# andimarafioti/faster-qwen3-tts

Hardware: AMD Instinct MI355X
Metric: real-time factor (audio s / wall s), Qwen3-TTS-12Hz-0.6B voice-clone streaming chunk_size=8; p50 TTFA in ttfa_ms_p50 (higher is better)
Workload: dtype bf16

## Files before the change

faster-qwen3-tts_amd/csrc/decode_kernels.cuh:

```cuda
#pragma once
#include "fq3_common.cuh"
#include <initializer_list>

namespace fq3 {

enum { PRO_PLAIN = 0, PRO_NORM = 1, PRO_COMBINE = 2 };
enum { EPI_STORE = 0, EPI_RESIDUAL = 1, EPI_SWIGLU = 2 };

constexpr int kHeadDim = 128;
constexpr int kKeysPerTile = 64;
constexpr int kMaxWorkers = 8;
constexpr int kPartStride = kHeadDim + 4;


struct GemvArgs {
    const void* W; int N; int K;
    const void* x;
    const void* norm_w; float eps;
    const void* bias;
    void* y;
    const void* res;
    void* xn_out;
    int up_off;
    const float* part; int n_part; int rep;
    const void* x2; void* y2; const void* res2; size_t part_stride2;
};

struct CombineRegs {
    f32x4 oa[kMaxWorkers], ob[kMaxWorkers];
    float pm[kMaxWorkers], pl[kMaxWorkers];
};
__device__ __forceinline__ void combine_load(CombineRegs& c, const float* part, int e0, int rep, int n_part) {
    const int head = e0 / kHeadDim, d0 = e0 - head * kHeadDim;
    const int g = head / rep, hh = head - g * rep;
    const float* p0 = part + ((size_t)(g * kMaxWorkers) * rep + hh) * kPartStride;
    const size_t sstride = (size_t)rep * kPartStride;
#pragma unroll
    for (int s = 0; s < kMaxWorkers; ++s) {
        const float* ps = p0 + (s < n_part ? s : 0) * sstride;
        c.oa[s] = *reinterpret_cast<const f32x4*>(ps + d0);
        c.ob[s] = *reinterpret_cast<const f32x4*>(ps + d0 + 4);
        c.pm[s] = ps[kHeadDim]; c.pl[s] = ps[kHeadDim + 1];
    }
}
template <typename T>
__device__ __forceinline__ void combine_finish(CombineRegs& c, int n_part, float (&f)[8]) {
#pragma unroll
    for (int s = 1; s < kMaxWorkers; ++s)
        if (s >= n_part) { c.pm[s] = -1e30f; c.pl[s] = 0.f; }
    float Mx = c.pm[0];
#pragma unroll
    for (int s = 1; s < kMaxWorkers; ++s) Mx = fmaxf(Mx, c.pm[s]);
    f32x4 na = f32x4{0.f, 0.f, 0.f, 0.f}, nb = na;
    float den = 0.f;
#pragma unroll
    for (int s = 0; s < kMaxWorkers; ++s) {
        const float w = __expf(c.pm[s] - Mx);
        na += c.oa[s] * w; nb += c.ob[s] * w; den = fmaf(w, c.pl[s], den);
    }
    const float inv = 1.0f / den;
    f[0] = na.x * inv; f[1] = na.y * inv; f[2] = na.z * inv; f[3] = na.w * inv;
    f[4] = nb.x * inv; f[5] = nb.y * inv; f[6] = nb.z * inv; f[7] = nb.w * inv;
#pragma unroll
    for (int i = 0; i < 8; i += 2) DT<T>::rnd2(f[i], f[i + 1]);
}

template <int NCH, int EPI> struct MaxRows {
    static constexpr int NR = EPI == EPI_SWIGLU ? 2 : 1;
    static constexpr int v = NCH >= 12 ? 1 : (NCH >= 6 ? (2 / NR) : 2);
};

inline int gemv_chunks(int K, int most) {
    const int need = (K + 511) / 512;
    for (int n : {1, 2, 4, 6, 12}) if (need <= n && n <= most) return n;
    return 0;
}

template <typename T, int NCH, int PRO, int EPI, bool NT, int M = 1, int R = 1>
__device__ __forceinline__ void gemv_body(const GemvArgs& a) {
    constexpr int NR = (EPI == EPI_SWIGLU) ? 2 : 1;
    extern __shared__ __attribute__((aligned(16))) float xs[];
    const int tid = threadIdx.x, wave = tid >> 6, lane = tid & 63;
    const int K = a.K;
    const T* W = reinterpret_cast<const T*>(a.W);
    const int row0 = (blockIdx.x * 4 + wave) * R;

    Raw8<T> xraw[M][NCH], nraw[NCH];
    CombineRegs cr[M];
    if constexpr (PRO == PRO_COMBINE) {
        const int e0 = tid * 8 < K ? tid * 8 : 0;
#pragma unroll
        for (int m = 0; m < M; ++m) combine_load(cr[m], a.part + (size_t)m * a.part_stride2, e0, a.rep, a.n_part);
    } else {
#pragma unroll
        for (int j = 0; j < NCH; ++j) {
            const int off = j * 512 + lane * 8, offc = off < K ? off : 0;
#pragma unroll
            for (int m = 0; m < M; ++m) ldraw<false>(xraw[m][j], reinterpret_cast<const T*>(m == 0 ? a.x : a.x2) + offc);
            if constexpr (PRO == PRO_NORM) ldraw<false>(nraw[j], reinterpret_cast<const T*>(a.norm_w) + offc);
        }
    }
    __builtin_amdgcn_sched_barrier(0);

    Raw8<T> raw[NR][R][NCH];
#pragma unroll
    for (int h = 0; h < NR; ++h)
#pragma unroll
        for (int r = 0; r < R; ++r) {
            const int row = row0 + r < a.N ? row0 + r : a.N - 1;
            const T* wr = W + (size_t)(row + h * a.up_off) * K;
#pragma unroll
            for (int j = 0; j < NCH; ++j) {
                const int off = j * 512 + lane * 8;
                ldraw<NT>(raw[h][r][j], wr + (off < K ? off : 0));
            }
        }
    float resv[M][R], biasv[R];
#pragma unroll
    for (int r = 0; r < R; ++r) {
        const int row = row0 + r < a.N ? row0 + r : a.N - 1;
#pragma unroll
        for (int m = 0; m < M; ++m) {
            const T* rp = reinterpret_cast<const T*>(m == 0 ? a.res : a.res2);
            resv[m][r] = 0.f;
            if constexpr (EPI == EPI_RESIDUAL) resv[m][r] = DT<T>::ld(rp + row);
        }
        const T* bp = a.bias ? reinterpret_cast<const T*>(a.bias) + row : W;
        const float bv = DT<T>::ld(bp);
        biasv[r] = a.bias ? bv : 0.f;
    }
    __builtin_amdgcn_sched_barrier(0);

    float xr[M][NCH][8];
    if constexpr (PRO == PRO_COMBINE) {
#pragma unroll
        for (int m = 0; m < M; ++m) {
            float f[8];
            combine_finish<T>(cr[m], a.n_part, f);
            if (tid * 8 < K) {
                float* d = xs + (size_t)m * K + tid * 8;
                reinterpret_cast<f32x4*>(d)[0] = f32x4{f[0], f[1], f[2], f[3]};
                reinterpret_cast<f32x4*>(d)[1] = f32x4{f[4], f[5], f[6], f[7]};
            }
        }
        __syncthreads();
#pragma unroll
        for (int m = 0; m < M; ++m)
#pragma unroll
            for (int j = 0; j < NCH; ++j) {
                const int off = j * 512 + lane * 8, offc = off < K ? off : 0;
                const float z = off < K ? 1.f : 0.f;
                const f32x4 lo = *reinterpret_cast<const f32x4*>(xs + (size_t)m * K + offc) * z;
                const f32x4 hi = *reinterpret_cast<const f32x4*>(xs + (size_t)m * K + offc + 4) * z;
                xr[m][j][0] = lo.x; xr[m][j][1] = lo.y; xr[m][j][2] = lo.z; xr[m][j][3] = lo.w;
                xr[m][j][4] = hi.x; xr[m][j][5] = hi.y; xr[m][j][6] = hi.z; xr[m][j][7] = hi.w;
            }
    } else {
#pragma unroll
        for (int m = 0; m < M; ++m) {
#pragma unroll
            for (int j = 0; j < NCH; ++j) {
                if (j * 512 + lane * 8 >= K) zero(xraw[m][j]);
                unpack(xraw[m][j], xr[m][j]);
            }
            if constexpr (PRO == PRO_NORM) {
                float ss = 0.f;
#pragma unroll
                for (int j = 0; j < NCH; ++j)
#pragma unroll
                    for (int i = 0; i < 8; ++i) ss = fmaf(xr[m][j][i], xr[m][j][i], ss);
                ss = wave_sum(ss);
                const float rs = 1.0f / sqrtf(ss / (float)K + a.eps);
#pragma unroll
                for (int j = 0; j < NCH; ++j) {
                    float nw[8];
                    unpack(nraw[j], nw);
#pragma unroll
                    for (int i = 0; i < 8; i += 2) {
                        float u = xr[m][j][i] * rs, v = xr[m][j][i + 1] * rs;
                        DT<T>::rnd2(u, v);
                        u *= nw[i]; v *= nw[i + 1];
                        DT<T>::rnd2(u, v);
                        xr[m][j][i] = u; xr[m][j][i + 1] = v;
                    }
                }
            }
        }
    }

    float acc[M][R][NR];
#pragma unroll
    for (int m = 0; m < M; ++m)
#pragma unroll
        for (int r = 0; r < R; ++r)
#pragma unroll
            for (int h = 0; h < NR; ++h) {
                float s = 0.f;
#pragma unroll
                for (int j = 0; j < NCH; ++j) s = dot8<T>(raw[h][r][j], xr[m][j], s);
                acc[m][r][h] = s;
            }
#pragma unroll
    for (int m = 0; m < M; ++m)
#pragma unroll
        for (int r = 0; r < R; ++r)
#pragma unroll
            for (int h = 0; h < NR; ++h) acc[m][r][h] = wave_sum(acc[m][r][h]);
#pragma unroll
    for (int r = 0; r < R; ++r) {
        const int row = row0 + r;
#pragma unroll
        for (int m = 0; m < M; ++m) {
            float v;
            if constexpr (EPI == EPI_SWIGLU) {
                const float g = DT<T>::rnd(acc[m][r][0]);
                const float u = DT<T>::rnd(acc[m][r][NR - 1]);
                const float sg = DT<T>::rnd(g / (1.0f + expf(-g)));
                v = sg * u;
            } else {
                v = DT<T>::rnd(acc[m][r][0] + biasv[r]);
                if constexpr (EPI == EPI_RESIDUAL) v = v + resv[m][r];
            }
            if (lane == 0 && row < a.N) DT<T>::st(reinterpret_cast<T*>(m == 0 ? a.y : a.y2) + row, v);
        }
    }
    if (a.xn_out && blockIdx.x == 0 && wave == 0) {
        T* o = reinterpret_cast<T*>(a.xn_out);
#pragma unroll
        for (int j = 0; j < NCH; ++j) {
            const int off = j * 512 + lane * 8;
            if (off < K) DT<T>::st8(o + off, xr[0][j]);
        }
    }
}

template <typename T, int NCH, int PRO, int EPI, bool NT, int M = 1, int R = 1>
__global__ __launch_bounds__(256) void gemv_kernel(GemvArgs a) { gemv_body<T, NCH, PRO, EPI, NT, M, R>(a); }

struct AttnArgs {
    const void* qkv;
    const void* q_norm_w; const void* k_norm_w; float eps;
    const float* cos_row; const float* sin_row;
    void* kcache; void* vcache; int max_seq;
    const int* table; int blk_stride;
    const int* pos_ptr; int pos_imm; int n_pad;
    const int* done_ptr;
    int n_kv; float* part; float scale;
    int rep; void* out;
};

template <typename T, int REP, bool PAGED>
__device__ __forceinline__ void attn_decode_body(const AttnArgs& a) {
    constexpr int HD = kHeadDim, KS = kKeysPerTile, NG = KS / 16;
    const int g = blockIdx.x, s = blockIdx.y, S = gridDim.y;
    __shared__ float qs[REP][HD];
    __shared__ float knew[HD], vnew[HD];
    __shared__ float wo[4][REP][HD];
    __shared__ float wm[4][REP], wl[4][REP];
    const int tid = threadIdx.x, wave = tid >> 6, lane = tid & 63;
    const int sub = lane >> 4, c = lane & 15;
    const T* qkv = reinterpret_cast<const T*>(a.qkv);
    const int q_dim = a.n_kv * REP * HD, kv_dim = a.n_kv * HD;
    T* kc = reinterpret_cast<T*>(a.kcache) + (PAGED ? (size_t)g * KS * HD : (size_t)g * a.max_seq * HD);
    T* vc = reinterpret_cast<T*>(a.vcache) + (PAGED ? (size_t)g * KS * HD : (size_t)g * a.max_seq * HD);
    const int n_tiles = (a.max_seq + KS - 1) / KS;
    auto block_of = [&](int tile) -> int {
        if constexpr (PAGED) return a.table[tile < n_tiles ? tile : n_tiles - 1];
        else return 0;
    };
    int blk = block_of(s), blk_next = block_of(s + S);

    Raw8<T> kr[NG], vr[NG];
    auto issue_tile = [&](int tile, int b) {
#pragma unroll
        for (int i = 0; i < NG; ++i) {
            const int kt = (i * 4 + wave) * 4 + sub;
            size_t off;
            if constexpr (PAGED) off = (size_t)b * a.blk_stride + (size_t)kt * HD;
            else { int key = tile * KS + kt; key = key < a.max_seq ? key : a.max_seq - 1; off = (size_t)key * HD; }
            ldraw<false>(kr[i], kc + off + c * 8);
            ldraw<false>(vr[i], vc + off + c * 8);
        }
    };
    if constexpr (!PAGED) issue_tile(s, 0);
    constexpr int NV = (REP + 2 + 3) / 4;
    float px0[NV], px1[NV], pw0[NV], pw1[NV];
#pragma unroll
    for (int i = 0; i < NV; ++i) {
        const int vec = wave + 4 * i < REP + 2 ? wave + 4 * i : REP + 1;
        const T* src = vec < REP ? qkv + (size_t)(g * REP + vec) * HD
                     : (vec == REP ? qkv + q_dim + (size_t)g * HD : qkv + q_dim + kv_dim + (size_t)g * HD);
        px0[i] = DT<T>::ld(src + lane); px1[i] = DT<T>::ld(src + lane + 64);
        const T* w = reinterpret_cast<const T*>(vec < REP ? a.q_norm_w : a.k_norm_w);
        pw0[i] = DT<T>::ld(w + lane); pw1[i] = DT<T>::ld(w + lane + 64);
    }
    const float cs = a.cos_row[lane], sn = a.sin_row[lane];
    const int pos = a.pos_ptr ? *a.pos_ptr : a.pos_imm;
    const int done_word = *(a.done_ptr ? a.done_ptr : reinterpret_cast<const int*>(a.cos_row));
    const bool loop_done = a.done_ptr != nullptr && done_word != 0;
    if constexpr (PAGED) issue_tile(s, blk);
    __builtin_amdgcn_sched_barrier(0);

    const int t_pos = pos / KS;
    const bool owner = (t_pos % S) == s;
    const bool may_append = owner && !loop_done;
    size_t new_off = (size_t)pos * HD;
    if constexpr (PAGED) new_off = (size_t)block_of(t_pos) * a.blk_stride + (size_t)(pos - t_pos * KS) * HD;
#pragma unroll
    for (int i = 0; i < NV; ++i) {
        const int vec = wave + 4 * i;
        if (vec >= REP + 2) continue;
        float x0 = px0[i], x1 = px1[i];
        if (vec <= REP) {
            const float ss = wave_sum(fmaf(x0, x0, x1 * x1));
            const float rs = 1.0f / sqrtf(ss / (float)HD + a.eps);
            const float n0 = DT<T>::rnd(pw0[i] * DT<T>::rnd(x0 * rs));
            const float n1 = DT<T>::rnd(pw1[i] * DT<T>::rnd(x1 * rs));
            x0 = DT<T>::rnd(DT<T>::rnd(n0 * cs) + DT<T>::rnd(-n1 * sn));
            x1 = DT<T>::rnd(DT<T>::rnd(n1 * cs) + DT<T>::rnd(n0 * sn));
        }
        if (vec < REP) { qs[vec][lane] = x0; qs[vec][lane + 64] = x1; }
        else {
            float* dst = vec == REP ? knew : vnew;
            dst[lane] = x0; dst[lane + 64] = x1;
            if (may_append) {
                T* cp = (vec == REP ? kc : vc) + new_off;
                DT<T>::st(cp + lane, x0); DT<T>::st(cp + lane + 64, x1);
            }
        }
    }
    __syncthreads();

    float qr[REP][8];
#pragma unroll
    for (int h = 0; h < REP; ++h)
#pragma unroll
        for (int i = 0; i < 8; ++i) qr[h][i] = qs[h][c * 8 + i];

    float m[REP], l[REP], o[REP][8];
#pragma unroll
    for (int h = 0; h < REP; ++h) {
        m[h] = -1e30f; l[h] = 0.f;
#pragma unroll
        for (int i = 0; i < 8; ++i) o[h][i] = 0.f;
    }
    auto step = [&](const float (&kf)[8], const float (&vf)[8], bool valid) {
#pragma unroll
        for (int h = 0; h < REP; ++h) {
            float sc = 0.f;
#pragma unroll
            for (int i = 0; i < 8; ++i) sc = fmaf(qr[h][i], kf[i], sc);
            sc = row16_sum(sc);
            sc = valid ? sc * a.scale : -INFINITY;
            const float mn = fmaxf(m[h], sc);
            const float al = __expf(m[h] - mn);
            const float p = __expf(sc - mn);
            l[h] = fmaf(l[h], al, p);
#pragma unroll
            for (int i = 0; i < 8; ++i) o[h][i] = fmaf(o[h][i], al, valid ? p * vf[i] : 0.f);
            m[h] = mn;
        }
    };
    for (int tile = s; tile * KS < pos || tile == s; tile += S) {
        if (tile != s) { blk = blk_next; issue_tile(tile, blk); }
        blk_next = block_of(tile + S);
#pragma unroll
        for (int i = 0; i < NG; ++i) {
            const int key = tile * KS + (i * 4 + wave) * 4 + sub;
            float kf[8], vf[8];
            unpack(kr[i], kf); unpack(vr[i], vf);
            step(kf, vf, key >= a.n_pad && key < pos);
        }
    }
    {
        float kf[8], vf[8];
#pragma unroll
        for (int i = 0; i < 8; ++i) { kf[i] = knew[c * 8 + i]; vf[i] = vnew[c * 8 + i]; }
        step(kf, vf, owner && wave == 0 && sub == 0 && pos >= a.n_pad);
    }
#pragma unroll
    for (int h = 0; h < REP; ++h) {
        const float M = xrow_max(m[h]);
        const float w = __expf(m[h] - M);
        l[h] = xrow_sum(l[h] * w);
#pragma unroll
        for (int i = 0; i < 8; ++i) o[h][i] = xrow_sum(o[h][i] * w);
        m[h] = M;
    }
    if (sub == 0) {
#pragma unroll
        for (int h = 0; h < REP; ++h) {
#pragma unroll
            for (int i = 0; i < 8; ++i) wo[wave][h][c * 8 + i] = o[h][i];
            if (c == 0) { wm[wave][h] = m[h]; wl[wave][h] = l[h]; }
        }
    }
    __syncthreads();
    for (int e = tid; e < REP * HD; e += 256) {
        const int h = e / HD, d = e - h * HD;
        float M = fmaxf(fmaxf(wm[0][h], wm[1][h]), fmaxf(wm[2][h], wm[3][h]));
        float num = 0.f, den = 0.f;
#pragma unroll
        for (int w = 0; w < 4; ++w) {
            const float ww = __expf(wm[w][h] - M);
            num = fmaf(ww, wo[w][h][d], num);
            den = fmaf(ww, wl[w][h], den);
        }
        float* p = a.part + (((size_t)g * kMaxWorkers + s) * REP + h) * kPartStride;
        p[d] = num;
        if (d == 0) { p[HD] = M; p[HD + 1] = den; }
    }
}

template <typename T, int REP, bool PAGED>
__global__ __launch_bounds__(256) void attn_decode_kernel(AttnArgs a) { attn_decode_body<T, REP, PAGED>(a); }

template <typename T>
__device__ __forceinline__ void attn_pred_body(const AttnArgs& a, int head) {
    constexpr int HD = kHeadDim;
    const int g = head / a.rep, hh = head - g * a.rep;
    const int lane = threadIdx.x & 63, sub = lane >> 4, c = lane & 15;
    const int pos = a.pos_imm;
    const T* qkv = reinterpret_cast<const T*>(a.qkv);
    const int q_dim = a.n_kv * a.rep * HD, kv_dim = a.n_kv * HD;
    T* kc = reinterpret_cast<T*>(a.kcache) + (size_t)g * a.max_seq * HD;
    T* vc = reinterpret_cast<T*>(a.vcache) + (size_t)g * a.max_seq * HD;
    Raw8<T> qraw, knraw, vnraw, qwraw, kwraw, kr[4], vr[4];
    ldraw<false>(qraw, qkv + (size_t)head * HD + c * 8);
    ldraw<false>(knraw, qkv + q_dim + (size_t)g * HD + c * 8);
    ldraw<false>(vnraw, qkv + q_dim + kv_dim + (size_t)g * HD + c * 8);
    ldraw<false>(qwraw, reinterpret_cast<const T*>(a.q_norm_w) + c * 8);
    ldraw<false>(kwraw, reinterpret_cast<const T*>(a.k_norm_w) + c * 8);
    const f32x4 cs0 = *reinterpret_cast<const f32x4*>(a.cos_row + ((c * 8) & 63)), cs1 = *reinterpret_cast<const f32x4*>(a.cos_row + ((c * 8 + 4) & 63));
    const f32x4 sn0 = *reinterpret_cast<const f32x4*>(a.sin_row + ((c * 8) & 63)), sn1 = *reinterpret_cast<const f32x4*>(a.sin_row + ((c * 8 + 4) & 63));
#pragma unroll
    for (int i = 0; i < 4; ++i) {
        int key = i * 4 + sub;
        key = key < a.max_seq ? key : a.max_seq - 1;
        ldraw<false>(kr[i], kc + (size_t)key * HD + c * 8);
        ldraw<false>(vr[i], vc + (size_t)key * HD + c * 8);
    }
    __builtin_amdgcn_sched_barrier(0);
    const float sgn = c < 8 ? -1.f : 1.f;
    const float cs[8] = {cs0.x, cs0.y, cs0.z, cs0.w, cs1.x, cs1.y, cs1.z, cs1.w};
    const float sn[8] = {sgn * sn0.x, sgn * sn0.y, sgn * sn0.z, sgn * sn0.w, sgn * sn1.x, sgn * sn1.y, sgn * sn1.z, sgn * sn1.w};
    auto norm_rope = [&](const Raw8<T>& raw, const Raw8<T>& wraw, float (&out)[8]) {
        float x[8], w[8];
        unpack(raw, x); unpack(wraw, w);
        float ss = 0.f;
#pragma unroll
        for (int i = 0; i < 8; ++i) ss = fmaf(x[i], x[i], ss);
        ss = row16_sum(ss);
        const float rs = 1.0f / sqrtf(ss / (float)HD + a.eps);
#pragma unroll
        for (int i = 0; i < 8; i += 2) {
            float u = x[i] * rs, v = x[i + 1] * rs;
            DT<T>::rnd2(u, v);
            u *= w[i]; v *= w[i + 1];
            DT<T>::rnd2(u, v);
            x[i] = u; x[i + 1] = v;
        }
#pragma unroll
        for (int i = 0; i < 8; i += 2) {
            float a0 = x[i] * cs[i], a1 = x[i + 1] * cs[i + 1];
            float b0 = row16_xor8(x[i]) * sn[i], b1 = row16_xor8(x[i + 1]) * sn[i + 1];
            DT<T>::rnd2(a0, a1); DT<T>::rnd2(b0, b1);
            float r0 = a0 + b0, r1 = a1 + b1;
            DT<T>::rnd2(r0, r1);
            out[i] = r0; out[i + 1] = r1;
        }
    };
    float qr[8], knew[8], vnew[8];
    norm_rope(qraw, qwraw, qr);
    norm_rope(knraw, kwraw, knew);
    unpack(vnraw, vnew);
    if (hh == 0 && sub == 0) {
        DT<T>::st8(kc + (size_t)pos * HD + c * 8, knew);
        DT<T>::st8(vc + (size_t)pos * HD + c * 8, vnew);
    }
    float sc[5];
#pragma unroll
    for (int i = 0; i < 4; ++i) {
        float kf[8], s = 0.f;
        unpack(kr[i], kf);
#pragma unroll
        for (int d = 0; d < 8; ++d) s = fmaf(qr[d], kf[d], s);
        s = row16_sum(s);
        sc[i] = (i * 4 + sub < pos) ? s * a.scale : -INFINITY;
    }
    {
        float s = 0.f;
#pragma unroll
        for (int d = 0; d < 8; ++d) s = fmaf(qr[d], knew[d], s);
        s = row16_sum(s);
        sc[4] = sub == 0 ? s * a.scale : -INFINITY;
    }
    const float mx = wave_max(fmaxf(fmaxf(fmaxf(sc[0], sc[1]), fmaxf(sc[2], sc[3])), sc[4]));
    float p[5], lsum = 0.f, o[8];
#pragma unroll
    for (int i = 0; i < 5; ++i) { p[i] = __expf(sc[i] - mx); lsum += p[i]; }
    lsum = wave_sum(lsum) * (1.0f / 16.0f);
#pragma unroll
    for (int d = 0; d < 8; ++d) o[d] = p[4] * vnew[d];
#pragma unroll
    for (int i = 0; i < 4; ++i) {
        float vf[8];
        if (!(i * 4 + sub < pos)) zero(vr[i]);
        unpack(vr[i], vf);
#pragma unroll
        for (int d = 0; d < 8; ++d) o[d] = fmaf(p[i], vf[d], o[d]);
    }
    const float inv = 1.0f / lsum;
#pragma unroll
    for (int d = 0; d < 8; ++d) o[d] = xrow_sum(o[d]) * inv;
    if (sub == 0) DT<T>::st8(reinterpret_cast<T*>(a.out) + (size_t)head * HD + c * 8, o);
}

template <typename T>
__device__ __forceinline__ void attn_pred_body(const AttnArgs& a) { attn_pred_body<T>(a, (int)blockIdx.x); }

template <typename T, int REP>
__device__ __forceinline__ void attn_pred_group_body(const AttnArgs& a, int g) {
    constexpr int HD = kHeadDim;
    const int lane = threadIdx.x & 63, sub = lane >> 4, c = lane & 15;
    const int pos = a.pos_imm;
    const T* qkv = reinterpret_cast<const T*>(a.qkv);
    const int q_dim = a.n_kv * REP * HD, kv_dim = a.n_kv * HD;
    T* kc = reinterpret_cast<T*>(a.kcache) + (size_t)g * a.max_seq * HD;
    T* vc = reinterpret_cast<T*>(a.vcache) + (size_t)g * a.max_seq * HD;
    Raw8<T> qraw[REP], knraw, vnraw, qwraw, kwraw, kr[4], vr[4];
#pragma unroll
    for (int h = 0; h < REP; ++h) ldraw<false>(qraw[h], qkv + (size_t)(g * REP + h) * HD + c * 8);
    ldraw<false>(knraw, qkv + q_dim + (size_t)g * HD + c * 8);
    ldraw<false>(vnraw, qkv + q_dim + kv_dim + (size_t)g * HD + c * 8);
    ldraw<false>(qwraw, reinterpret_cast<const T*>(a.q_norm_w) + c * 8);
    ldraw<false>(kwraw, reinterpret_cast<const T*>(a.k_norm_w) + c * 8);
    const f32x4 cs0 = *reinterpret_cast<const f32x4*>(a.cos_row + ((c * 8) & 63)), cs1 = *reinterpret_cast<const f32x4*>(a.cos_row + ((c * 8 + 4) & 63));
    const f32x4 sn0 = *reinterpret_cast<const f32x4*>(a.sin_row + ((c * 8) & 63)), sn1 = *reinterpret_cast<const f32x4*>(a.sin_row + ((c * 8 + 4) & 63));
#pragma unroll
    for (int i = 0; i < 4; ++i) {
        int key = i * 4 + sub;
        key = key < pos ? key : 0;
        ldraw<false>(kr[i], kc + (size_t)key * HD + c * 8);
        ldraw<false>(vr[i], vc + (size_t)key * HD + c * 8);
    }
    __builtin_amdgcn_sched_barrier(0);
    const float sgn = c < 8 ? -1.f : 1.f;
    const float cs[8] = {cs0.x, cs0.y, cs0.z, cs0.w, cs1.x, cs1.y, cs1.z, cs1.w};
    const float sn[8] = {sgn * sn0.x, sgn * sn0.y, sgn * sn0.z, sgn * sn0.w, sgn * sn1.x, sgn * sn1.y, sgn * sn1.z, sgn * sn1.w};
    auto norm_rope = [&](const Raw8<T>& raw, const Raw8<T>& wraw, float (&out)[8]) {
        float x[8], w[8];
        unpack(raw, x); unpack(wraw, w);
        float ss = 0.f;
#pragma unroll
        for (int i = 0; i < 8; ++i) ss = fmaf(x[i], x[i], ss);
        ss = row16_sum(ss);
        const float rs = 1.0f / sqrtf(ss / (float)HD + a.eps);
#pragma unroll
        for (int i = 0; i < 8; i += 2) {
            float u = x[i] * rs, v = x[i + 1] * rs;
            DT<T>::rnd2(u, v);
            u *= w[i]; v *= w[i + 1];
            DT<T>::rnd2(u, v);
            x[i] = u; x[i + 1] = v;
        }
#pragma unroll
        for (int i = 0; i < 8; i += 2) {
            float a0 = x[i] * cs[i], a1 = x[i + 1] * cs[i + 1];
            float b0 = row16_xor8(x[i]) * sn[i], b1 = row16_xor8(x[i + 1]) * sn[i + 1];
            DT<T>::rnd2(a0, a1); DT<T>::rnd2(b0, b1);
            float r0 = a0 + b0, r1 = a1 + b1;
            DT<T>::rnd2(r0, r1);
            out[i] = r0; out[i + 1] = r1;
        }
    };
    float knew[8], vnew[8];
    norm_rope(knraw, kwraw, knew);
    unpack(vnraw, vnew);
    if (sub == 0) {
        DT<T>::st8(kc + (size_t)pos * HD + c * 8, knew);
        DT<T>::st8(vc + (size_t)pos * HD + c * 8, vnew);
    }
    float kf[4][8], vf[4][8];
#pragma unroll
    for (int i = 0; i < 4; ++i) {
        unpack(kr[i], kf[i]);
        if (!(i * 4 + sub < pos)) zero(vr[i]);
        unpack(vr[i], vf[i]);
    }
#pragma unroll
    for (int h = 0; h < REP; ++h) {
        float qr[8];
        norm_rope(qraw[h], qwraw, qr);
        float sc[5];
#pragma unroll
        for (int i = 0; i < 4; ++i) {
            float s = 0.f;
#pragma unroll
            for (int d = 0; d < 8; ++d) s = fmaf(qr[d], kf[i][d], s);
            s = row16_sum(s);
            sc[i] = (i * 4 + sub < pos) ? s * a.scale : -INFINITY;
        }
        {
            float s = 0.f;
#pragma unroll
            for (int d = 0; d < 8; ++d) s = fmaf(qr[d], knew[d], s);
            s = row16_sum(s);
            sc[4] = sub == 0 ? s * a.scale : -INFINITY;
        }
        const float mx = wave_max(fmaxf(fmaxf(fmaxf(sc[0], sc[1]), fmaxf(sc[2], sc[3])), sc[4]));
        float p[5], lsum = 0.f, o[8];
#pragma unroll
        for (int i = 0; i < 5; ++i) { p[i] = __expf(sc[i] - mx); lsum += p[i]; }
        lsum = wave_sum(lsum) * (1.0f / 16.0f);
#pragma unroll
        for (int d = 0; d < 8; ++d) o[d] = p[4] * vnew[d];
#pragma unroll
        for (int i = 0; i < 4; ++i)
#pragma unroll
            for (int d = 0; d < 8; ++d) o[d] = fmaf(p[i], vf[i][d], o[d]);
        const float inv = 1.0f / lsum;
#pragma unroll
        for (int d = 0; d < 8; ++d) o[d] = xrow_sum(o[d]) * inv;
        if (sub == 0) DT<T>::st8(reinterpret_cast<T*>(a.out) + (size_t)(g * REP + h) * HD + c * 8, o);
    }
}

template <typename T>
__global__ __launch_bounds__(64) void attn_pred_kernel(AttnArgs a) { attn_pred_body<T>(a); }

template <typename T>
__global__ __launch_bounds__(256) void rmsnorm_kernel(const T* x, const T* w, T* y, int K, float eps) {
    __shared__ float red[8];
    float ss = 0.f;
    for (int e = threadIdx.x; e < K; e += 256) { const float v = DT<T>::ld(x + e); ss = fmaf(v, v, ss); }
    ss = block_sum<4>(ss, red);
    const float rs = 1.0f / sqrtf(ss / (float)K + eps);
    for (int e = threadIdx.x; e < K; e += 256)
        DT<T>::st(y + e, DT<T>::ld(w + e) * DT<T>::rnd(DT<T>::ld(x + e) * rs));
}

template <typename T>
__global__ void copy_kernel(T* dst, const T* src, int n) {
    const int i = blockIdx.x * blockDim.x + threadIdx.x;
    if (i < n) dst[i] = src[i];
}

struct DecodeState {
    int token, frame, pos, gen_step, done;
    int text_open;
    int min_new, max_new, trailing_len, noise_frames, eos_id, max_seq, sup_lo, sup_hi;
    float t_temperature; int t_top_k; float t_top_p; int t_do_sample; float t_rep_penalty;
    float p_temperature; int p_top_k; float p_top_p; int p_do_sample;
    const void* trailing_text; const void* tts_pad; const void* talker_noise; const void* pred_noise;
    const void* past_hidden_init;
    int n_pad, rope_delta;
};

struct TeacherForcing { const int* forced; int* decisions; };

__device__ __forceinline__ int forced_or(const TeacherForcing* tf, int slot, int tok) {
    if (!tf) return tok;
    const int* forced = gptr(tf->forced); int* dec = gptr(tf->decisions);
    if (dec && threadIdx.x == 0) dec[slot] = tok;
    return forced ? forced[slot] : tok;
}

template <typename T>
__device__ __forceinline__ void frame_begin_body(DecodeState* st, const T* codec_emb, const T* past_hidden, T* ph_hold,
                                                 T* pred_in, int* codes, unsigned char* seen, int H, int G) {
    const int done = st->done;
    if (done == 1) return;
    const int tok = st->token;
    if (tok == st->eos_id || st->frame >= st->max_new) {
        __syncthreads();
        if (threadIdx.x == 0) st->done = 1;
        return;
    }
    if (st->text_open && st->gen_step >= st->trailing_len) {
        if (done == 0) {
            for (int e = threadIdx.x; e < H; e += 256) ph_hold[e] = past_hidden[e];
            __syncthreads();
            if (threadIdx.x == 0) st->done = 2;
        }
        return;
    }
    if (done == 2) {
        past_hidden = ph_hold;
        __syncthreads();
        if (threadIdx.x == 0) st->done = 0;
    }
    if (threadIdx.x == 0) { codes[(size_t)st->frame * G] = tok; seen[tok] = 1; }
    for (int e = threadIdx.x; e < H; e += 256) {
        pred_in[e] = past_hidden[e];
        pred_in[H + e] = codec_emb[(size_t)tok * H + e];
    }
}
template <typename T>
__global__ __launch_bounds__(256) void frame_begin_kernel(DecodeState* st, const T* codec_emb, const T* past_hidden, T* ph_hold,
                                                          T* pred_in, int* codes, unsigned char* seen, int H, int G) {
    frame_begin_body<T>(st, codec_emb, past_hidden, ph_hold, pred_in, codes, seen, H, G);
}

struct EmbTables { const void* t[32]; };

template <typename T, int G>
__device__ __forceinline__ void embed_sum_body(DecodeState* st, const EmbTables& tabs, const int* codes, T* x, int H,
                                               const float* cos_tab, const float* sin_tab, int rope_len,
                                               int rope_delta, float* rope_now) {
    const int done = st->done, frame = st->frame, pos = st->pos, gen_step = st->gen_step;
    const int trailing_len = st->trailing_len, max_seq = st->max_seq;
    const T* trailing = gptr(reinterpret_cast<const T*>(st->trailing_text));
    const T* pad = gptr(reinterpret_cast<const T*>(st->tts_pad));
    if (done) return;
    if (pos >= max_seq - 1) {
        __syncthreads();
        if (threadIdx.x == 0) { st->frame = frame + 1; st->done = 1; }
        return;
    }
    int ids[G];
#pragma unroll
    for (int gI = 0; gI < G; ++gI) ids[gI] = codes[(size_t)frame * G + gI];
    if (threadIdx.x < kHeadDim) {
        int rp = pos + rope_delta;
        rp = rp < 0 ? 0 : (rp >= rope_len ? rope_len - 1 : rp);
        const int i = threadIdx.x & 63;
        rope_now[threadIdx.x] = threadIdx.x < 64 ? cos_tab[(size_t)rp * 64 + i] : sin_tab[(size_t)rp * 64 + i];
    }
    const T* text = gen_step < trailing_len ? trailing + (size_t)gen_step * H : pad;
    for (int e0 = threadIdx.x * 8; e0 < H; e0 += 256 * 8) {
        Raw8<T> r[G], tr;
#pragma unroll
        for (int gI = 0; gI < G; ++gI) ldraw<false>(r[gI], reinterpret_cast<const T*>(tabs.t[gI]) + (size_t)ids[gI] * H + e0);
        ldraw<false>(tr, text + e0);
        float sum[8], f[8];
        unpack(r[0], sum);
#pragma unroll
        for (int gI = 1; gI < G; ++gI) {
            unpack(r[gI], f);
#pragma unroll
            for (int i = 0; i < 8; ++i) sum[i] += f[i];
        }
        unpack(tr, f);
#pragma unroll
        for (int i = 0; i < 8; ++i) DT<T>::st(x + e0 + i, DT<T>::rnd(sum[i]) + f[i]);
    }
}
template <typename T, int G>
__global__ __launch_bounds__(256) void embed_sum_kernel(DecodeState* st, EmbTables tabs, const int* codes, T* x, int H,
                                                        const float* cos_tab, const float* sin_tab, int rope_len,
                                                        int rope_delta, float* rope_now) {
    embed_sum_body<T, G>(st, tabs, codes, x, H, cos_tab, sin_tab, rope_len, rope_delta, rope_now);
}

}
```

faster-qwen3-tts_amd/csrc/fq3_api.hip:

```cpp
#define FQ3_SKINNY_EXTERN
#include "fq3_ctx.h"
#include "sampler.cuh"
#include "sampler_wave.cuh"
#include "skinny_gemm.cuh"

#include <cstdio>
#include <cstdlib>
#include <cstring>
#include <map>
#include <string>
#include <type_traits>
#include <vector>

using namespace fq3;

static thread_local std::string g_err;
static int fail(int code, const std::string& m) { g_err = m; return code; }
int fq3_fail_(int code, const std::string& m) { return fail(code, m); }
#define HIPCHK(x) do { hipError_t e_ = (x); if (e_ != hipSuccess) return fail(FQ3_EHIP, std::string(#x) + ": " + hipGetErrorString(e_)); } while (0)

extern "C" const char* fq3_last_error(void) { return g_err.c_str(); }
extern "C" void fq3_set_error_(const char* msg) { g_err = msg ? msg : ""; }
extern "C" int fq3_abi_version(void) { return FQ3_ABI_VERSION; }

static int dmalloc(fq3_ctx* c, void** p, size_t bytes, bool zero = true) {
    HIPCHK(hipMalloc(p, bytes));
    if (zero) HIPCHK(hipMemset(*p, 0, bytes));
    c->allocs.push_back(*p);
    return 0;
}
int fq3_dmalloc_(fq3_ctx* c, void** p, size_t bytes) { return dmalloc(c, p, bytes, false); }

static bool dims_ok(const fq3_stack_dims& d) {
    return d.head_dim == kHeadDim && d.hidden % 8 == 0 && d.inter % 8 == 0 && d.n_heads % d.n_kv_heads == 0 &&
           (d.n_heads / d.n_kv_heads == 1 || d.n_heads / d.n_kv_heads == 2 || d.n_heads / d.n_kv_heads == 4) &&
           d.vocab <= kMaxVocab && d.vocab % 8 == 0 && d.hidden <= 2048 && d.inter <= 6144 && d.n_heads * kHeadDim <= 6144 && d.n_layers >= 1;
}

static int cfg_check(const fq3_config* cfg) {
    if (cfg->dtype != FQ3_BF16 && cfg->dtype != FQ3_F32) return fail(FQ3_EINVAL, "dtype must be FQ3_BF16 or FQ3_F32");
    if (!dims_ok(cfg->talker) || !dims_ok(cfg->predictor))
        return fail(FQ3_EUNSUPPORTED, "unsupported dims (need head_dim 128, GQA ratio 1/2/4, vocab <= 4096 and a multiple of 8, "
                                      "hidden <= 2048 and intermediate <= 6144, both multiples of 8)");
    if (cfg->num_code_groups < 2 || cfg->num_code_groups > 64) return fail(FQ3_EINVAL, "num_code_groups");
    if (cfg->max_seq_len < 8) return fail(FQ3_EINVAL, "max_seq_len");
    return 0;
}

static void pool_free_(fq3_kv_pool* p) {
    for (void* q : p->k) if (q) (void)hipFree(q);
    for (void* q : p->v) if (q) (void)hipFree(q);
    delete p;
}

static int pool_create_(const fq3_config* cfg, int n_blocks, fq3_kv_pool** out) {
    if (n_blocks < 1) return fail(FQ3_EINVAL, "fq3_kv_pool_create: n_blocks must be positive");
    fq3_kv_pool* p = new fq3_kv_pool();
    p->dtype = cfg->dtype; p->esz = cfg->dtype == FQ3_BF16 ? 2 : 4;
    p->n_layers = cfg->talker.n_layers; p->n_kv = cfg->talker.n_kv_heads; p->n_blocks = n_blocks;
    p->blk_elems = (size_t)p->n_kv * kKeysPerTile * kHeadDim;
    p->k.assign(p->n_layers, nullptr); p->v.assign(p->n_layers, nullptr);
    const size_t bytes = (size_t)n_blocks * p->blk_elems * p->esz;
    for (int i = 0; i < p->n_layers; ++i) {
        if (hipMalloc(&p->k[i], bytes) != hipSuccess || hipMalloc(&p->v[i], bytes) != hipSuccess ||
            hipMemset(p->k[i], 0, bytes) != hipSuccess || hipMemset(p->v[i], 0, bytes) != hipSuccess) {
            pool_free_(p);
            return fail(FQ3_EHIP, "fq3_kv_pool_create: allocation of " + std::to_string(2 * bytes >> 20) + " MiB per layer failed");
        }
    }
    p->free_list.resize(n_blocks);
    for (int i = 0; i < n_blocks; ++i) p->free_list[i] = n_blocks - 1 - i;
    *out = p;
    return FQ3_OK;
}

extern "C" int fq3_kv_pool_create(const fq3_config* cfg, int n_blocks, fq3_kv_pool** out) {
    if (!cfg || !out) return fail(FQ3_EINVAL, "null argument");
    if (int r = cfg_check(cfg)) return r;
    return pool_create_(cfg, n_blocks, out);
}

extern "C" int fq3_kv_pool_destroy(fq3_kv_pool* p) {
    if (!p) return FQ3_OK;
    if (p->users > 0) return fail(FQ3_ESTATE, "fq3_kv_pool_destroy: contexts are still attached");
    (void)hipDeviceSynchronize();
    pool_free_(p);
    return FQ3_OK;
}

extern "C" int fq3_kv_pool_stats(const fq3_kv_pool* p, int* n_blocks, int* n_free, int* high_water, int64_t* bytes_per_block) {
    if (!p) return fail(FQ3_EINVAL, "null pool");
    fq3_kv_pool* q = const_cast<fq3_kv_pool*>(p);
    std::lock_guard<std::mutex> lk(q->mu);
    if (n_blocks) *n_blocks = p->n_blocks;
    if (n_free) *n_free = (int)p->free_list.size();
    if (high_water) *high_water = p->in_use_high;
    if (bytes_per_block) *bytes_per_block = (int64_t)2 * p->n_layers * p->blk_elems * p->esz;
    return FQ3_OK;
}

struct KvTableVals { int v[128]; };
__global__ void kv_table_write_kernel(int* table, KvTableVals vals, int first, int count) {
    const int i = threadIdx.x;
    if (i < count) table[first + i] = vals.v[i];
}
static void table_write(fq3_ctx* c, const int* ids, int first, int count, hipStream_t s) {
    for (int o = 0; o < count; o += 128) {
        KvTableVals t{};
        const int n = std::min(128, count - o);
        for (int i = 0; i < n; ++i) t.v[i] = ids[o + i];
        hipLaunchKernelGGL(kv_table_write_kernel, dim3(1), dim3(128), 0, s, c->tk.d_table, t, first + o, n);
    }
}

static int kv_ensure(fq3_ctx* c, int n_pos, hipStream_t s, bool sync_copy);
int fq3_kv_ensure_(fq3_ctx* c, int n_pos, hipStream_t s) { return kv_ensure(c, n_pos, s, false); }
static int kv_ensure(fq3_ctx* c, int n_pos, hipStream_t s, bool sync_copy) {
    StackBufs& b = c->tk;
    int need = (std::min(n_pos, b.max_seq) + kKeysPerTile - 1) / kKeysPerTile;
    need = std::min(need, b.max_blocks);
    const int have = (int)b.blocks.size();
    if (need <= have) return 0;
    fq3_kv_pool* p = b.pool;
    {
        std::lock_guard<std::mutex> lk(p->mu);
        if ((int)p->free_list.size() < need - have) {
            char m[200];
            snprintf(m, sizeof m, "KV pool exhausted: %d more block(s) of 64 keys needed, %d free of %d", need - have, (int)p->free_list.size(), p->n_blocks);
            return fail(FQ3_ENOMEM, m);
        }
        for (int i = have; i < need; ++i) { b.blocks.push_back(p->free_list.back()); p->free_list.pop_back(); }
        p->in_use_high = std::max(p->in_use_high, p->n_blocks - (int)p->free_list.size());
    }
    if (sync_copy) HIPCHK(hipMemcpy(b.d_table + have, b.blocks.data() + have, (size_t)(need - have) * sizeof(int), hipMemcpyHostToDevice));
    else table_write(c, b.blocks.data() + have, have, need - have, s);
    return 0;
}

extern "C" int fq3_kv_release(fq3_ctx* c, int keep_positions) {
    if (!c) return fail(FQ3_EINVAL, "null ctx");
    StackBufs& b = c->tk;
    const int keep = std::max(0, std::min((int)b.blocks.size(), (keep_positions + kKeysPerTile - 1) / kKeysPerTile));
    if (keep >= (int)b.blocks.size()) return FQ3_OK;
    std::lock_guard<std::mutex> lk(b.pool->mu);
    while ((int)b.blocks.size() > keep) { b.pool->free_list.push_back(b.blocks.back()); b.blocks.pop_back(); }
    return FQ3_OK;
}

extern "C" int fq3_kv_blocks(const fq3_ctx* c) { return c ? (int)c->tk.blocks.size() : 0; }

extern "C" int fq3_kv_reserve(fq3_ctx* c, int n_positions, void* stream) {
    if (!c) return fail(FQ3_EINVAL, "null ctx");
    if (n_positions < 0) return fail(FQ3_EINVAL, "fq3_kv_reserve: negative position count");
    return fq3_kv_ensure_(c, n_positions, (hipStream_t)stream);
}

static int ctx_build(fq3_ctx* c, const fq3_config* cfg, fq3_kv_pool* pool);
static int ctx_create_(const fq3_config* cfg, fq3_kv_pool* pool, fq3_ctx** out) {
    if (!cfg || !out) return fail(FQ3_EINVAL, "null argument");
    if (int r = cfg_check(cfg)) return r;
    if (pool && (pool->dtype != cfg->dtype || pool->n_layers != cfg->talker.n_layers || pool->n_kv != cfg->talker.n_kv_heads))
        return fail(FQ3_EINVAL, "fq3_ctx_create_pooled: the pool was built for another dtype / layer count / kv head count");
    fq3_ctx* c = new fq3_ctx();
    if (int r = ctx_build(c, cfg, pool)) { const std::string m = g_err; fq3_ctx_destroy(c); g_err = m; return r; }
    *out = c;
    return FQ3_OK;
}
extern "C" int fq3_ctx_create(const fq3_config* cfg, fq3_ctx** out) { return ctx_create_(cfg, nullptr, out); }
extern "C" int fq3_ctx_create_pooled(const fq3_config* cfg, fq3_kv_pool* pool, fq3_ctx** out) {
    if (!pool) return fail(FQ3_EINVAL, "null pool");
    return ctx_create_(cfg, pool, out);
}

static int ctx_build(fq3_ctx* c, const fq3_config* cfg, fq3_kv_pool* pool) {
    c->cfg = *cfg;
    c->esz = cfg->dtype == FQ3_BF16 ? 2 : 4;
    const fq3_stack_dims &t = cfg->talker, &p = cfg->predictor;
    const int pred_seq = cfg->num_code_groups + 1;
    auto alloc_stack = [&](StackBufs& b, const fq3_stack_dims& d, int max_seq) -> int {
        b.max_seq = max_seq;
        b.workers = std::min(kMaxWorkers, (max_seq + kKeysPerTile - 1) / kKeysPerTile);
        b.k.resize(d.n_layers); b.v.resize(d.n_layers);
        const size_t bytes = (size_t)d.n_kv_heads * max_seq * kHeadDim * c->esz;
        for (int i = 0; i < d.n_layers; ++i) {
            if (int r = dmalloc(c, &b.k[i], bytes)) return r;
            if (int r = dmalloc(c, &b.v[i], bytes)) return r;
        }
        return 0;
    };
    int r;
    {
        StackBufs& b = c->tk;
        b.max_seq = cfg->max_seq_len;
        b.max_blocks = (cfg->max_seq_len + kKeysPerTile - 1) / kKeysPerTile;
        b.workers = std::min(kMaxWorkers, b.max_blocks);
        if (!pool) {
            if ((r = pool_create_(cfg, b.max_blocks, &pool))) return r;
            pool->is_private = true;
        }
        b.pool = pool;
        { std::lock_guard<std::mutex> lk(pool->mu); ++pool->users; }
        b.k = pool->k; b.v = pool->v;
        if ((r = dmalloc(c, (void**)&b.d_table, (size_t)b.max_blocks * sizeof(int)))) return r;
        if (pool->is_private && (r = kv_ensure(c, cfg->max_seq_len, nullptr, true))) return r;
    }
    if ((r = alloc_stack(c->pk, p, pred_seq))) return r;
    const int Hm = std::max(t.hidden, p.hidden), Im = std::max(t.inter, p.inter);
    const int qkvm = std::max(t.n_heads + 2 * t.n_kv_heads, p.n_heads + 2 * p.n_kv_heads) * kHeadDim;
    const int Vm = std::max(t.vocab, p.vocab);
    const int G = cfg->num_code_groups;
    const int frames = cfg->max_frames > 0 ? cfg->max_frames : 4096;
    c->cfg.max_frames = frames;
    if ((r = dmalloc(c, &c->h, (size_t)Hm * c->esz))) return r;
    if ((r = dmalloc(c, &c->h2, (size_t)Hm * c->esz))) return r;
    if ((r = dmalloc(c, &c->qkv2, (size_t)qkvm * c->esz))) return r;
    if ((r = dmalloc(c, &c->attn_out, (size_t)qkvm * c->esz))) return r;
    if ((r = dmalloc(c, &c->attn_out2, (size_t)qkvm * c->esz))) return r;
    if ((r = dmalloc(c, &c->act2, (size_t)Im * c->esz))) return r;
    if ((r = dmalloc(c, &c->pred_x2, (size_t)p.hidden * c->esz))) return r;
    if ((r = dmalloc(c, &c->xin, (size_t)Hm * c->esz))) return r;
    if ((r = dmalloc(c, &c->tmp_hidden, (size_t)Hm * c->esz))) return r;
    if ((r = dmalloc(c, &c->qkv, (size_t)qkvm * c->esz))) return r;
    if ((r = dmalloc(c, &c->act, (size_t)Im * c->esz))) return r;
    if ((r = dmalloc(c, &c->logits, (size_t)Vm * c->esz))) return r;
    if ((r = dmalloc(c, &c->past_hidden, (size_t)t.hidden * c->esz))) return r;
    if ((r = dmalloc(c, &c->ph_hold, (size_t)t.hidden * c->esz))) return r;
    if ((r = dmalloc(c, &c->pred_in, (size_t)2 * t.hidden * c->esz))) return r;
    if ((r = dmalloc(c, &c->pred_next, (size_t)t.hidden * c->esz))) return r;
    if ((r = dmalloc(c, &c->pred_x, (size_t)p.hidden * c->esz))) return r;
    if ((r = dmalloc(c, &c->plogits, (size_t)(G - 1) * p.vocab * c->esz))) return r;
    const int maxkv = std::max(t.n_kv_heads, p.n_kv_heads);
    c->part_stride = (size_t)maxkv * kMaxWorkers * 4 * kPartStride;
    if ((r = dmalloc(c, (void**)&c->part, 2 * c->part_stride * sizeof(float)))) return r;
    if ((r = dmalloc(c, (void**)&c->rope_now, 2 * 64 * sizeof(float)))) return r;
    if ((r = dmalloc(c, (void**)&c->seen_api, kMaxVocab))) return r;
    if ((r = dmalloc(c, (void**)&c->st, sizeof(DecodeState)))) return r;
    if ((r = dmalloc(c, (void**)&c->seen, kMaxVocab))) return r;
    if ((r = dmalloc(c, (void**)&c->codes, (size_t)(frames + 1) * G * sizeof(int)))) return r;
    if ((r = dmalloc(c, (void**)&c->ids64, (size_t)64 * sizeof(int64_t)))) return r;
    if ((r = dmalloc(c, (void**)&c->d_pemb, (size_t)64 * sizeof(void*)))) return r;
    HIPCHK(hipStreamCreateWithFlags(&c->cap_stream, hipStreamNonBlocking));
    return FQ3_OK;
}

extern "C" int fq3_set_option(fq3_ctx* c, const char* key, int value) {
    if (!c || !key) return fail(FQ3_EINVAL, "null argument");
    const std::string k(key);
    if (k == "weight_nt") c->opt_nt = value;
    else if (k == "pred_m2") c->opt_m2 = value;
    else if (k == "pred_attn") c->opt_pred_attn = value;
    else if (k == "rows_per_wave_max") c->opt_rmax = value;
    else if (k == "prefill_mode") c->prefill_mode = value;
    else if (k == "flash_prefill") c->opt_flash_prefill = value;
    else if (k == "flash_small") c->opt_flash_small = value;
    else if (k == "swiglu_tile") c->opt_swiglu_tile = value;
    else if (k == "packed_weights") c->opt_packed = value;
    else if (k == "skinny_gemm") c->opt_no_skinny = !value;
    else return fail(FQ3_EINVAL, "unknown option: " + k);
    fq3_graph_reset(c);
    return FQ3_OK;
}

extern "C" int fq3_graph_reset(fq3_ctx* c) {
    if (!c) return fail(FQ3_EINVAL, "null ctx");
    if (c->exec) { (void)hipGraphExecDestroy(c->exec); c->exec = nullptr; }
    if (c->graph) { (void)hipGraphDestroy(c->graph); c->graph = nullptr; }
    return FQ3_OK;
}

namespace {
struct PackedEntry { void* p; int refs; int N, K; };
std::mutex g_packed_mu;
std::map<std::pair<const void*, int>, PackedEntry> g_packed;
}
const void* fq3_packed_find_(const void* W, int kind) {
    std::lock_guard<std::mutex> lk(g_packed_mu);
    auto it = g_packed.find({W, kind});
    return it == g_packed.end() ? nullptr : it->second.p;
}
int fq3_packed_acquire_(const void* W, int N, int K, int kind) {
    if (!W || !skinny_pack_ok(N, K) || (kind == 1 && (N / 2) % 8) || (kind == 2 && N % 512)) return FQ3_EUNSUPPORTED;
    std::lock_guard<std::mutex> lk(g_packed_mu);
    auto it = g_packed.find({W, kind});
    if (it != g_packed.end()) {
        if (it->second.N != N || it->second.K != K) return fail(FQ3_EINVAL, "a matrix is bound with two different shapes");
        ++it->second.refs;
        return FQ3_OK;
    }
    void* p = nullptr;
    if (hipMalloc(&p, (size_t)N * K * 2) != hipSuccess) { (void)hipGetLastError(); return fail(FQ3_ENOMEM, "no device memory for the fragment-major weight copy"); }
    skinny_pack(reinterpret_cast<const bf16_t*>(W), reinterpret_cast<bf16_t*>(p), N, K, kind == 1 ? N / 2 : (kind == 2 ? -(N / 2) : 0), nullptr);
    if (hipStreamSynchronize(nullptr) != hipSuccess) { (void)hipFree(p); return fail(FQ3_EHIP, "packing a weight matrix failed"); }
    g_packed[{W, kind}] = PackedEntry{p, 1, N, K};
    return FQ3_OK;
}
void fq3_packed_release_(const void* W, int kind) {
    std::lock_guard<std::mutex> lk(g_packed_mu);
    auto it = g_packed.find({W, kind});
    if (it == g_packed.end()) return;
    if (--it->second.refs <= 0) { (void)hipFree(it->second.p); g_packed.erase(it); }
}
static void packed_release_all(fq3_ctx* c) {
    for (auto& r : c->packed_refs) fq3_packed_release_(r.first, r.second);
    c->packed_refs.clear();
}
static int packed_acquire_all(fq3_ctx* c) {
    if (c->cfg.dtype != FQ3_BF16) return FQ3_OK;
    auto take = [&](const void* W, int N, int K, int kind) -> int {
        const int r = fq3_packed_acquire_(W, N, K, kind);
        if (r == FQ3_OK) c->packed_refs.emplace_back(W, kind);
        return r == FQ3_EUNSUPPORTED ? FQ3_OK : r;
    };
    auto stack = [&](const std::vector<fq3_layer_weights>& L, const fq3_stack_dims& d) -> int {
        const int qd = d.n_heads * kHeadDim, kvd = d.n_kv_heads * kHeadDim;
        for (const fq3_layer_weights& l : L) {
            if (int r = take(l.qkv, qd + 2 * kvd, d.hidden, 0)) return r;
            if (int r = take(l.o, d.hidden, qd, 0)) return r;
            if (int r = take(l.gate_up, 2 * d.inter, d.hidden, 1)) return r;
            if (int r = take(l.gate_up, 2 * d.inter, d.hidden, 0)) return r;
            if (int r = take(l.down, d.hidden, d.inter, 0)) return r;
        }
        return FQ3_OK;
    };
    if (int r = stack(c->tl, c->cfg.talker)) return r;
    if (int r = stack(c->pl, c->cfg.predictor)) return r;
    for (const fq3_layer_weights& l : c->tl) if (int r = take(l.gate_up, 2 * c->cfg.talker.inter, c->cfg.talker.hidden, 2)) return r;
    if (int r = take(c->wt.codec_head, c->cfg.talker.vocab, c->cfg.talker.hidden, 0)) return r;
    for (const void* h : c->lmh) if (int r = take(h, c->cfg.predictor.vocab, c->cfg.predictor.hidden, 0)) return r;
    return FQ3_OK;
}

extern "C" int fq3_ctx_destroy(fq3_ctx* c) {
    if (!c) return FQ3_OK;
    (void)hipDeviceSynchronize();
    fq3_graph_reset(c);
    packed_release_all(c);
    if (c->cap_stream) (void)hipStreamDestroy(c->cap_stream);
    if (fq3_kv_pool* p = c->tk.pool) {
        (void)fq3_kv_release(c, 0);
        bool last;
        { std::lock_guard<std::mutex> lk(p->mu); last = --p->users == 0; }
        if (p->is_private && last) pool_free_(p);
    }
    for (void* p : c->allocs) (void)hipFree(p);
    delete c;
    return FQ3_OK;
}

extern "C" int fq3_bind_weights(fq3_ctx* c, const fq3_weight_table* w) {
    if (!c || !w) return fail(FQ3_EINVAL, "null argument");
    const int G = c->cfg.num_code_groups;
    if (!w->talker_layers || !w->predictor_layers || !w->codec_embedding || !w->codec_head || !w->talker_final_norm ||
        !w->predictor_final_norm || !w->predictor_embeddings || !w->lm_heads || !w->talker_cos || !w->talker_sin ||
        !w->pred_cos || !w->pred_sin)
        return fail(FQ3_EINVAL, "weight table has null entries");
    if (c->cfg.has_projection && !w->proj_w) return fail(FQ3_EINVAL, "has_projection set but proj_w is null");
    if (w->talker_rope_len < c->cfg.max_seq_len || w->pred_rope_len < G + 1)
        return fail(FQ3_EINVAL, "rope tables shorter than the caches");
    c->wt = *w;
    c->tl.assign(w->talker_layers, w->talker_layers + c->cfg.talker.n_layers);
    c->pl.assign(w->predictor_layers, w->predictor_layers + c->cfg.predictor.n_layers);
    c->pemb.assign(w->predictor_embeddings, w->predictor_embeddings + (G - 1));
    c->lmh.assign(w->lm_heads, w->lm_heads + (G - 1));
    for (auto& l : c->tl) if (!l.qkv || !l.o || !l.gate_up || !l.down || !l.input_norm || !l.post_norm || !l.q_norm || !l.k_norm)
        return fail(FQ3_EINVAL, "talker layer has null weights");
    for (auto& l : c->pl) if (!l.qkv || !l.o || !l.gate_up || !l.down || !l.input_norm || !l.post_norm || !l.q_norm || !l.k_norm)
        return fail(FQ3_EINVAL, "predictor layer has null weights");
    HIPCHK(hipMemcpy(c->d_pemb, c->pemb.data(), (G - 1) * sizeof(void*), hipMemcpyHostToDevice));
    (void)hipDeviceSynchronize();
    packed_release_all(c);
    if (int r = packed_acquire_all(c)) { packed_release_all(c); return r; }
    c->bound = true;
    fq3_graph_reset(c);
    return FQ3_OK;
}

template <typename T, int NCH, int PRO, int EPI, bool NT, int M = 1>
static void launch_gemv_n(const GemvArgs& a, int rmax, hipStream_t s) {
    int R = (a.N + 1023) / 1024;
    if (R > MaxRows<NCH, EPI>::v) R = MaxRows<NCH, EPI>::v;
    if (rmax > 0 && R > rmax) R = rmax;
    if (R < 1) R = 1;
    const int grid = (a.N + 4 * R - 1) / (4 * R);
    const size_t shm = PRO == PRO_COMBINE ? (size_t)M * a.K * sizeof(float) : 0;
    if constexpr (MaxRows<NCH, EPI>::v >= 2) {
        if (R == 2) { hipLaunchKernelGGL((gemv_kernel<T, NCH, PRO, EPI, NT, M, 2>), dim3(grid), dim3(256), shm, s, a); return; }
    }
    hipLaunchKernelGGL((gemv_kernel<T, NCH, PRO, EPI, NT, M, 1>), dim3(grid), dim3(256), shm, s, a);
}
template <typename T, int PRO, int EPI>
static int launch_gemv2_t(const GemvArgs& a, int rmax, hipStream_t s) {
    constexpr int most = PRO == PRO_NORM ? 4 : 6;
    const int n = gemv_chunks(a.K, most);
    if (!n) return fail(FQ3_EUNSUPPORTED, PRO == PRO_NORM ? "code predictor hidden size above 2048" : "code predictor GEMV inner dimension above 3072");
    with_value<1, 2, 4, 6>(n, [&](auto nch) {
        if constexpr (decltype(nch)::value <= most) launch_gemv_n<T, decltype(nch)::value, PRO, EPI, false, 2>(a, rmax, s);
    });
    return 0;
}
template <int PRO, int EPI>
static int launch_gemv2(const fq3_ctx* c, const GemvArgs& a, hipStream_t s) {
    return c->cfg.dtype == FQ3_BF16 ? launch_gemv2_t<bf16_t, PRO, EPI>(a, c->opt_rmax, s) : launch_gemv2_t<float, PRO, EPI>(a, c->opt_rmax, s);
}
template <typename T, int PRO, int EPI, bool NT>
static int launch_gemv_t(const GemvArgs& a, int rmax, hipStream_t s) {
    constexpr int most = PRO == PRO_NORM ? 4 : 12;
    const int n = gemv_chunks(a.K, most);
    if (!n) return fail(FQ3_EUNSUPPORTED, PRO == PRO_NORM ? "hidden size above 2048" : "GEMV inner dimension above 6144");
    with_value<1, 2, 4, 6, 12>(n, [&](auto nch) {
        if constexpr (decltype(nch)::value <= most) launch_gemv_n<T, decltype(nch)::value, PRO, EPI, NT>(a, rmax, s);
    });
    return 0;
}
template <int PRO, int EPI>
static int launch_gemv(const fq3_ctx* c, const GemvArgs& a, bool nt, hipStream_t s) {
    const int rmax = c->opt_rmax;
    if (c->cfg.dtype == FQ3_BF16)
        return nt ? launch_gemv_t<bf16_t, PRO, EPI, true>(a, rmax, s) : launch_gemv_t<bf16_t, PRO, EPI, false>(a, rmax, s);
    return nt ? launch_gemv_t<float, PRO, EPI, true>(a, rmax, s) : launch_gemv_t<float, PRO, EPI, false>(a, rmax, s);
}

template <typename T, bool PAGED>
static void launch_attn_p(const AttnArgs& a, int rep, int workers, hipStream_t s) {
    with_value<1, 2, 4>(rep, [&](auto r) {
        hipLaunchKernelGGL((attn_decode_kernel<T, decltype(r)::value, PAGED>), dim3(a.n_kv, workers), dim3(256), 0, s, a);
    });
}
template <typename T>
static void launch_attn_t(const AttnArgs& a, int rep, int workers, hipStream_t s) {
    if (a.table) launch_attn_p<T, true>(a, rep, workers, s); else launch_attn_p<T, false>(a, rep, workers, s);
}

struct StepSrc { const void* x0; const int* pos_ptr; int pos_imm; bool kv_only_tail = false; };

static int run_stack(fq3_ctx* c, bool talker, const StepSrc& src, hipStream_t s) {
    const fq3_stack_dims& d = talker ? c->cfg.talker : c->cfg.predictor;
    const std::vector<fq3_layer_weights>& L = talker ? c->tl : c->pl;
    StackBufs& kv = talker ? c->tk : c->pk;
    const int rep = d.n_heads / d.n_kv_heads;
    const int q_dim = d.n_heads * kHeadDim, kv_dim = d.n_kv_heads * kHeadDim;
    const bool nt = c->opt_nt == 2 || (c->opt_nt == 1 && talker);
    const float *cos_row, *sin_row;
    if (src.pos_ptr) { cos_row = c->rope_now; sin_row = c->rope_now + 64; }
    else {
        const int rl = talker ? c->wt.talker_rope_len : c->wt.pred_rope_len;
        int rp = src.pos_imm + (talker ? c->rope_delta : 0);
        rp = rp < 0 ? 0 : (rp >= rl ? rl - 1 : rp);
        cos_row = (talker ? c->wt.talker_cos : c->wt.pred_cos) + (size_t)rp * 64;
        sin_row = (talker ? c->wt.talker_sin : c->wt.pred_sin) + (size_t)rp * 64;
    }
    for (int i = 0; i < d.n_layers; ++i) {
        const fq3_layer_weights& w = L[i];
        const void* xin = i == 0 ? src.x0 : c->h;
        GemvArgs g{};
        g.eps = d.rms_eps;
        g.W = w.qkv; g.N = q_dim + 2 * kv_dim; g.K = d.hidden; g.x = xin;
        g.norm_w = w.input_norm; g.y = c->qkv;
        if (int r = launch_gemv<PRO_NORM, EPI_STORE>(c, g, nt, s)) return r;
        const bool tail_skip = src.kv_only_tail && i == d.n_layers - 1;
        GemvArgs o{};
        o.W = w.o; o.N = d.hidden; o.K = q_dim; o.y = c->h; o.res = xin; o.rep = rep;
        AttnArgs a{};
        a.qkv = c->qkv; a.q_norm_w = w.q_norm; a.k_norm_w = w.k_norm; a.eps = d.rms_eps;
        a.cos_row = cos_row; a.sin_row = sin_row;
        a.kcache = kv.k[i]; a.vcache = kv.v[i]; a.max_seq = kv.max_seq;
        a.table = kv.d_table; a.blk_stride = kv.pool ? (int)kv.pool->blk_elems : 0;
        a.pos_ptr = src.pos_ptr; a.pos_imm = src.pos_imm;
        a.done_ptr = src.pos_ptr ? &c->st->done : nullptr;
        a.n_pad = talker ? c->n_pad : 0;
        a.n_kv = d.n_kv_heads; a.part = c->part;
        a.scale = 1.0f / sqrtf((float)kHeadDim);
        a.rep = rep; a.out = c->attn_out;
        const bool pred_attn = c->opt_pred_attn && !talker && !src.pos_ptr && src.pos_imm <= 16;
        if (pred_attn) {
            if (c->cfg.dtype == FQ3_BF16) hipLaunchKernelGGL((attn_pred_kernel<bf16_t>), dim3(d.n_heads), dim3(64), 0, s, a);
            else hipLaunchKernelGGL((attn_pred_kernel<float>), dim3(d.n_heads), dim3(64), 0, s, a);
            if (tail_skip) break;
            o.x = c->attn_out;
            if (int r = launch_gemv<PRO_PLAIN, EPI_RESIDUAL>(c, o, nt, s)) return r;
        } else {
            if (c->cfg.dtype == FQ3_BF16) launch_attn_t<bf16_t>(a, rep, kv.workers, s);
            else launch_attn_t<float>(a, rep, kv.workers, s);
            if (tail_skip) break;
            o.part = c->part; o.n_part = kv.workers;
            if (int r = launch_gemv<PRO_COMBINE, EPI_RESIDUAL>(c, o, nt, s)) return r;
        }
        GemvArgs m{};
        m.eps = d.rms_eps; m.W = w.gate_up; m.N = d.inter; m.K = d.hidden; m.x = c->h;
        m.norm_w = w.post_norm; m.y = c->act; m.up_off = d.inter;
        if (int r = launch_gemv<PRO_NORM, EPI_SWIGLU>(c, m, nt, s)) return r;
        GemvArgs dn{};
        dn.W = w.down; dn.N = d.hidden; dn.K = d.inter; dn.x = c->act; dn.y = c->h; dn.res = c->h;
        if (int r = launch_gemv<PRO_PLAIN, EPI_RESIDUAL>(c, dn, nt, s)) return r;
    }
    return 0;
}

static int run_predictor_pair(fq3_ctx* c, const void* x_a, const void* x_b, hipStream_t s) {
    const fq3_stack_dims& d = c->cfg.predictor;
    StackBufs& kv = c->pk;
    const int rep = d.n_heads / d.n_kv_heads;
    const int q_dim = d.n_heads * kHeadDim, kv_dim = d.n_kv_heads * kHeadDim;
    for (int i = 0; i < d.n_layers; ++i) {
        const fq3_layer_weights& w = c->pl[i];
        const void* xa = i == 0 ? x_a : c->h;
        const void* xb = i == 0 ? x_b : c->h2;
        GemvArgs g{};
        g.eps = d.rms_eps; g.W = w.qkv; g.N = q_dim + 2 * kv_dim; g.K = d.hidden; g.x = xa; g.x2 = xb;
        g.norm_w = w.input_norm; g.y = c->qkv; g.y2 = c->qkv2;
        if (int r = launch_gemv2<PRO_NORM, EPI_STORE>(c, g, s)) return r;
        for (int m = 0; m < 2; ++m) {
            AttnArgs a{};
            a.qkv = m == 0 ? c->qkv : c->qkv2; a.q_norm_w = w.q_norm; a.k_norm_w = w.k_norm; a.eps = d.rms_eps;
            a.cos_row = c->wt.pred_cos + (size_t)m * 64; a.sin_row = c->wt.pred_sin + (size_t)m * 64;
            a.kcache = kv.k[i]; a.vcache = kv.v[i]; a.max_seq = kv.max_seq;
            a.pos_ptr = nullptr; a.pos_imm = m; a.n_pad = 0; a.n_kv = d.n_kv_heads;
            a.part = c->part + (size_t)m * c->part_stride; a.scale = 1.0f / sqrtf((float)kHeadDim);
            a.rep = rep; a.out = m == 0 ? c->attn_out : c->attn_out2;
            if (c->opt_pred_attn) {
                if (c->cfg.dtype == FQ3_BF16) hipLaunchKernelGGL((attn_pred_kernel<bf16_t>), dim3(d.n_heads), dim3(64), 0, s, a);
                else hipLaunchKernelGGL((attn_pred_kernel<float>), dim3(d.n_heads), dim3(64), 0, s, a);
            } else if (c->cfg.dtype == FQ3_BF16) launch_attn_t<bf16_t>(a, rep, kv.workers, s);
            else launch_attn_t<float>(a, rep, kv.workers, s);
        }
        GemvArgs o{};
        o.W = w.o; o.N = d.hidden; o.K = q_dim; o.y = c->h; o.y2 = c->h2; o.res = xa; o.res2 = xb; o.rep = rep;
        if (c->opt_pred_attn) {
            o.x = c->attn_out; o.x2 = c->attn_out2;
            if (int r = launch_gemv2<PRO_PLAIN, EPI_RESIDUAL>(c, o, s)) return r;
        } else {
            o.part = c->part; o.part_stride2 = c->part_stride; o.n_part = kv.workers;
            if (int r = launch_gemv2<PRO_COMBINE, EPI_RESIDUAL>(c, o, s)) return r;
        }
        GemvArgs m{};
        m.eps = d.rms_eps; m.W = w.gate_up; m.N = d.inter; m.K = d.hidden; m.x = c->h; m.x2 = c->h2;
        m.norm_w = w.post_norm; m.y = c->act; m.y2 = c->act2; m.up_off = d.inter;
        if (int r = launch_gemv2<PRO_NORM, EPI_SWIGLU>(c, m, s)) return r;
        GemvArgs dn{};
        dn.W = w.down; dn.N = d.hidden; dn.K = d.inter; dn.x = c->act; dn.x2 = c->act2; dn.y = c->h; dn.y2 = c->h2;
        dn.res = c->h; dn.res2 = c->h2;
        if (int r = launch_gemv2<PRO_PLAIN, EPI_RESIDUAL>(c, dn, s)) return r;
    }
    return 0;
}

#define NEED_BOUND(c) do { if (!(c)) return fail(FQ3_EINVAL, "null ctx"); if (!(c)->bound) return fail(FQ3_ESTATE, "weights not bound"); } while (0)
#define LAUNCH_CHECK() HIPCHK(hipGetLastError())

extern "C" int fq3_set_generation_state(fq3_ctx* c, int n_pad, int rope_delta) {
    if (!c) return fail(FQ3_EINVAL, "null ctx");
    if (n_pad < 0 || n_pad >= c->cfg.max_seq_len) return fail(FQ3_EINVAL, "n_pad out of range");
    if (c->n_pad != n_pad || c->rope_delta != rope_delta) fq3_graph_reset(c);
    c->n_pad = n_pad; c->rope_delta = rope_delta;
    return FQ3_OK;
}

template <typename T, bool TO_CACHE>
__global__ __launch_bounds__(256) void kv_paged_copy_kernel(T* cache, const int* table, int blk_stride, T* dense, int n_kv, int L) {
    constexpr int EPC = 16 / (int)sizeof(T), CPR = kHeadDim / EPC;
    const int i = blockIdx.x * 256 + threadIdx.x;
    if (i >= n_kv * L * CPR) return;
    const int ch = i % CPR, row = i / CPR, key = row % L, h = row / L;
    T* cp = cache + (size_t)table[key / kKeysPerTile] * blk_stride + ((size_t)h * kKeysPerTile + key % kKeysPerTile) * kHeadDim + ch * EPC;
    T* dp = dense + ((size_t)h * L + key) * kHeadDim + ch * EPC;
    if (TO_CACHE) *reinterpret_cast<u32x4*>(cp) = *reinterpret_cast<const u32x4*>(dp);
    else *reinterpret_cast<u32x4*>(dp) = *reinterpret_cast<const u32x4*>(cp);
}
template <typename T, bool TO_CACHE>
static void kv_paged_copy(fq3_ctx* c, int layer, void* k, void* v, int L, hipStream_t s) {
    const int nk = c->cfg.talker.n_kv_heads, n = nk * L * (kHeadDim * (int)sizeof(T) / 16);
    if (n <= 0) return;
    const int bs = (int)c->tk.pool->blk_elems;
    hipLaunchKernelGGL((kv_paged_copy_kernel<T, TO_CACHE>), dim3((n + 255) / 256), dim3(256), 0, s, (T*)c->tk.k[layer], c->tk.d_table, bs, (T*)k, nk, L);
    hipLaunchKernelGGL((kv_paged_copy_kernel<T, TO_CACHE>), dim3((n + 255) / 256), dim3(256), 0, s, (T*)c->tk.v[layer], c->tk.d_table, bs, (T*)v, nk, L);
}

extern "C" int fq3_kv_import(fq3_ctx* c, int layer, const void* k, const void* v, int L, void* stream) {
    if (!c || !k || !v) return fail(FQ3_EINVAL, "null argument");
    if (layer < 0 || layer >= c->cfg.talker.n_layers) return fail(FQ3_EINVAL, "layer out of range");
    if (L > c->cfg.max_seq_len) {
        char b[256];
        snprintf(b, sizeof b, "Input is too long: prefill has %d tokens but max_seq_len=%d. Use shorter text or shorter reference audio.",
                 L, c->cfg.max_seq_len);
        return fail(FQ3_ETOOLONG, b);
    }
    hipStream_t s = (hipStream_t)stream;
    if (int r = fq3_kv_ensure_(c, L, s)) return r;
    if (c->cfg.dtype == FQ3_BF16) kv_paged_copy<bf16_t, true>(c, layer, const_cast<void*>(k), const_cast<void*>(v), L, s);
    else kv_paged_copy<float, true>(c, layer, const_cast<void*>(k), const_cast<void*>(v), L, s);
    LAUNCH_CHECK();
    return FQ3_OK;
}

extern "C" int fq3_kv_export(fq3_ctx* c, int layer, void* k, void* v, int L, void* stream) {
    if (!c || !k || !v) return fail(FQ3_EINVAL, "null argument");
    if (layer < 0 || layer >= c->cfg.talker.n_layers || L > c->cfg.max_seq_len) return fail(FQ3_EINVAL, "range");
    if (L > (int)c->tk.blocks.size() * kKeysPerTile) return fail(FQ3_EINVAL, "fq3_kv_export: rows beyond the blocks this context owns");
    hipStream_t s = (hipStream_t)stream;
    if (c->cfg.dtype == FQ3_BF16) kv_paged_copy<bf16_t, false>(c, layer, k, v, L, s);
    else kv_paged_copy<float, false>(c, layer, k, v, L, s);
    LAUNCH_CHECK();
    return FQ3_OK;
}

struct KvAdoptTab { void* dst[128]; const void* src[128]; };
template <typename T>
__global__ __launch_bounds__(256) void kv_adopt_kernel(KvAdoptTab t, const int* dst_table, const int* src_table, int blk_elems) {
    const int which = blockIdx.x, b = blockIdx.y;
    const u32x4* s = reinterpret_cast<const u32x4*>(reinterpret_cast<const T*>(t.src[which]) + (size_t)src_table[b] * blk_elems);
    u32x4* d = reinterpret_cast<u32x4*>(reinterpret_cast<T*>(t.dst[which]) + (size_t)dst_table[b] * blk_elems);
    const int n16 = blk_elems * (int)sizeof(T) / 16;
    for (int i = threadIdx.x; i < n16; i += 256) d[i] = s[i];
}

extern "C" int fq3_kv_adopt(fq3_ctx* dst, fq3_ctx* src, int L, void* stream) {
    if (!dst || !src) return fail(FQ3_EINVAL, "null ctx");
    if (dst == src) return fail(FQ3_EINVAL, "fq3_kv_adopt: source and destination are the same context");
    const auto &a = dst->cfg, &b = src->cfg;
    if (a.dtype != b.dtype || a.talker.n_layers != b.talker.n_layers || a.talker.n_kv_heads != b.talker.n_kv_heads)
        return fail(FQ3_EINVAL, "fq3_kv_adopt: contexts of different shape");
    if (L < 0 || L > src->tk.max_seq || L > (int)src->tk.blocks.size() * kKeysPerTile) return fail(FQ3_EINVAL, "fq3_kv_adopt: L outside the source cache");
    if (L > dst->tk.max_seq) {
        char m[256];
        snprintf(m, sizeof m, "Input is too long: prefill has %d tokens but max_seq_len=%d. Use shorter text or shorter reference audio.", L, a.max_seq_len);
        return fail(FQ3_ETOOLONG, m);
    }
    const int nl = a.talker.n_layers;
    if (2 * nl > 128) return fail(FQ3_EUNSUPPORTED, "fq3_kv_adopt: more than 64 layers");
    if (L == 0) return FQ3_OK;
    hipStream_t s = (hipStream_t)stream;
    const int nb = (L + kKeysPerTile - 1) / kKeysPerTile;
    if (dst->tk.pool == src->tk.pool) {
        (void)fq3_kv_release(dst, 0);
        const size_t take = std::min(src->tk.blocks.size(), (size_t)dst->tk.max_blocks);
        dst->tk.blocks.assign(src->tk.blocks.begin(), src->tk.blocks.begin() + take);
        if (take < src->tk.blocks.size()) {
            std::lock_guard<std::mutex> lk(src->tk.pool->mu);
            for (size_t i = take; i < src->tk.blocks.size(); ++i) src->tk.pool->free_list.push_back(src->tk.blocks[i]);
        }
        src->tk.blocks.clear();
        table_write(dst, dst->tk.blocks.data(), 0, (int)take, s);
        LAUNCH_CHECK();
        return FQ3_OK;
    }
    if (int r = fq3_kv_ensure_(dst, L, s)) return r;
    KvAdoptTab t{};
    for (int l = 0; l < nl; ++l) { t.dst[2 * l] = dst->tk.k[l]; t.src[2 * l] = src->tk.k[l]; t.dst[2 * l + 1] = dst->tk.v[l]; t.src[2 * l + 1] = src->tk.v[l]; }
    const dim3 grid(2 * nl, nb);
    const int be = (int)dst->tk.pool->blk_elems;
    if (a.dtype == FQ3_BF16) hipLaunchKernelGGL((kv_adopt_kernel<bf16_t>), grid, dim3(256), 0, s, t, dst->tk.d_table, src->tk.d_table, be);
    else hipLaunchKernelGGL((kv_adopt_kernel<float>), grid, dim3(256), 0, s, t, dst->tk.d_table, src->tk.d_table, be);
    LAUNCH_CHECK();
    return FQ3_OK;
}

static int final_norm(fq3_ctx* c, bool talker, const void* x, void* y, hipStream_t s) {
    const fq3_stack_dims& d = talker ? c->cfg.talker : c->cfg.predictor;
    const void* w = talker ? c->wt.talker_final_norm : c->wt.predictor_final_norm;
    if (c->cfg.dtype == FQ3_BF16)
        hipLaunchKernelGGL((rmsnorm_kernel<bf16_t>), dim3(1), dim3(256), 0, s, (const bf16_t*)x, (const bf16_t*)w, (bf16_t*)y, d.hidden, d.rms_eps);
    else
        hipLaunchKernelGGL((rmsnorm_kernel<float>), dim3(1), dim3(256), 0, s, (const float*)x, (const float*)w, (float*)y, d.hidden, d.rms_eps);
    return 0;
}

extern "C" int fq3_talker_step(fq3_ctx* c, const void* embeds, int position, void* out_hidden, void* stream) {
    NEED_BOUND(c);
    if (!embeds || !out_hidden) return fail(FQ3_EINVAL, "null argument");
    if (position < 0 || position >= c->cfg.max_seq_len) return fail(FQ3_EINVAL, "position outside the static cache");
    hipStream_t s = (hipStream_t)stream;
    if (int r = fq3_kv_ensure_(c, position + 1, s)) return r;
    StepSrc src{embeds, nullptr, position};
    if (int r = run_stack(c, true, src, s)) return r;
    final_norm(c, true, c->h, out_hidden, s);
    LAUNCH_CHECK();
    return FQ3_OK;
}

extern "C" int fq3_codec_head(fq3_ctx* c, const void* hidden, void* out_logits, void* stream) {
    NEED_BOUND(c);
    if (!hidden || !out_logits) return fail(FQ3_EINVAL, "null argument");
    GemvArgs g{};
    g.W = c->wt.codec_head; g.N = c->cfg.talker.vocab; g.K = c->cfg.talker.hidden; g.x = hidden; g.y = out_logits;
    if (int r = launch_gemv<PRO_PLAIN, EPI_STORE>(c, g, true, (hipStream_t)stream)) return r;
    LAUNCH_CHECK();
    return FQ3_OK;
}

extern "C" int fq3_prefill(fq3_ctx* c, const void* embeds, int L, int n_pad, void* out_logits, void* out_hidden,
                           void* stream) {
    NEED_BOUND(c);
    if (!embeds || L <= 0) return fail(FQ3_EINVAL, "bad prompt");
    if (L > c->cfg.max_seq_len) {
        char b[256];
        snprintf(b, sizeof b, "Input is too long: prefill has %d tokens but max_seq_len=%d. Use shorter text or shorter reference audio.",
                 L, c->cfg.max_seq_len);
        return fail(FQ3_ETOOLONG, b);
    }
    if (n_pad < 0 || n_pad >= L) return fail(FQ3_EINVAL, "n_pad");
    if (int r = fq3_set_generation_state(c, n_pad, -n_pad)) return r;
    hipStream_t s = (hipStream_t)stream;
    if (int r = fq3_kv_ensure_(c, L, s)) return r;
    void* hid = out_hidden ? out_hidden : c->tmp_hidden;
    if (c->prefill_mode != 1 && L - n_pad >= 4) {
        if (int r = fq3_prefill_mfma_(c, embeds, L, n_pad, out_logits, hid, s)) return r;
        LAUNCH_CHECK();
        return FQ3_OK;
    }
    const size_t rowb = (size_t)c->cfg.talker.hidden * c->esz;
    for (int i = n_pad; i < L; ++i) {
        StepSrc src{(const char*)embeds + rowb * i, nullptr, i};
        if (int r = run_stack(c, true, src, s)) return r;
    }
    final_norm(c, true, c->h, hid, s);
    if (out_logits) {
        GemvArgs g{};
        g.W = c->wt.codec_head; g.N = c->cfg.talker.vocab; g.K = c->cfg.talker.hidden; g.x = hid; g.y = out_logits;
        if (int r = launch_gemv<PRO_PLAIN, EPI_STORE>(c, g, true, s)) return r;
    }
    LAUNCH_CHECK();
    return FQ3_OK;
}

extern "C" int fq3_prefill_reserve(fq3_ctx* c) {
    NEED_BOUND(c);
    return fq3_prefill_reserve_(c);
}

extern "C" int fq3_prefill_batch(fq3_ctx* const* ctxs, int n, const void* const* embeds, const int* L, const int* n_pad,
                                 void* const* out_logits, void* const* out_hidden, void* stream) {
    if (!ctxs || !embeds || !L || !n_pad || !out_hidden || n < 1 || n > 64) return fail(FQ3_EINVAL, "fq3_prefill_batch: bad argument");
    long total = 0;
    bool packed = true;
    for (int q = 0; q < n; ++q) {
        fq3_ctx* c = ctxs[q];
        NEED_BOUND(c);
        if (!embeds[q] || !out_hidden[q] || L[q] <= 0) return fail(FQ3_EINVAL, "fq3_prefill_batch: bad prompt");
        if (L[q] > c->cfg.max_seq_len) {
            char b[256];
            snprintf(b, sizeof b, "Input is too long: prefill has %d tokens but max_seq_len=%d. Use shorter text or shorter reference audio.",
                     L[q], c->cfg.max_seq_len);
            return fail(FQ3_ETOOLONG, b);
        }
        if (n_pad[q] < 0 || n_pad[q] >= L[q]) return fail(FQ3_EINVAL, "n_pad");
        total += L[q];
        const fq3_ctx* c0 = ctxs[0];
        packed = packed && c->cfg.dtype == c0->cfg.dtype && c->wt.codec_head == c0->wt.codec_head && c->tl.size() == c0->tl.size() &&
                 !c->tl.empty() && c->tl[0].qkv == c0->tl[0].qkv && c->prefill_mode != 1 && L[q] - n_pad[q] >= 4;
        for (int p = 0; p < q; ++p) if (ctxs[p] == c) return fail(FQ3_EINVAL, "fq3_prefill_batch: a context appears twice");
    }
    packed = packed && n > 1 && total <= ctxs[0]->cfg.max_seq_len;
    if (!packed) {
        for (int q = 0; q < n; ++q)
            if (int r = fq3_prefill(ctxs[q], embeds[q], L[q], n_pad[q], out_logits ? out_logits[q] : nullptr, out_hidden[q], stream)) return r;
        return FQ3_OK;
    }
    for (int q = 0; q < n; ++q)
        if (int r = fq3_set_generation_state(ctxs[q], n_pad[q], -n_pad[q])) return r;
    {
        std::vector<int> had(n);
        for (int q = 0; q < n; ++q) had[q] = (int)ctxs[q]->tk.blocks.size();
        for (int q = 0; q < n; ++q)
            if (int r = fq3_kv_ensure_(ctxs[q], L[q], (hipStream_t)stream)) {
                const std::string m = g_err;
                for (int p = 0; p < q; ++p) (void)fq3_kv_release(ctxs[p], had[p] * kKeysPerTile);
                g_err = m;
                return r;
            }
    }
    if (int r = fq3_prefill_batch_mfma_(ctxs, n, embeds, L, n_pad, out_logits, out_hidden, (hipStream_t)stream)) return r;
    LAUNCH_CHECK();
    return FQ3_OK;
}

int fq3_codec_head_launch_(fq3_ctx* c, const void* hidden, void* out_logits, hipStream_t s) {
    GemvArgs g{};
    g.W = c->wt.codec_head; g.N = c->cfg.talker.vocab; g.K = c->cfg.talker.hidden; g.x = hidden; g.y = out_logits;
    return launch_gemv<PRO_PLAIN, EPI_STORE>(c, g, true, s);
}

extern "C" int fq3_set_prefill_mode(fq3_ctx* c, int mode) { return fq3_set_option(c, "prefill_mode", mode); }

__global__ void build_seen_kernel(const int64_t* history, int n, unsigned char* seen, int V) {
    for (int i = threadIdx.x; i < V; i += blockDim.x) seen[i] = 0;
    __syncthreads();
    for (int i = threadIdx.x; i < n; i += blockDim.x) { const int id = (int)history[i]; if (id >= 0 && id < V) seen[id] = 1; }
}
template <typename F>
static void dispatch_nc(int V, F&& f) {
    if (V <= 2048) f(std::integral_constant<int, 1>{});
    else f(std::integral_constant<int, 2>{});
}

template <typename T>
static void launch_sample_pred(const DecodeState* st, const T* lg, int V, int cb, const SampleCfg& cfg, const T* nz,
                               int* codes, int G, int64_t* out64, const T* next_emb, T* next_in, int H, bool wave,
                               const TeacherForcing* tf, hipStream_t s) {
    if (wave) dispatch_nc(V, [&](auto nc) {
        constexpr int NC = decltype(nc)::value;
        hipLaunchKernelGGL((sample_pred_wave_kernel<T, NC>), dim3(1), dim3(256), 0, s, st, lg, V, cb, cfg, nz, codes, G,
                           out64, next_emb, next_in, H, tf);
    });
    else hipLaunchKernelGGL((sample_pred_kernel<T>), dim3(1), dim3(256), 0, s, st, lg, V, cb, cfg, nz, codes, G, out64,
                            next_emb, next_in, H, tf);
}
template <typename T>
static void launch_sample_talker(DecodeState* st, const T* lg, int V, const unsigned char* seen, int G, bool wave,
                                 const TeacherForcing* tf, hipStream_t s) {
    if (wave) dispatch_nc(V, [&](auto nc) {
        constexpr int NC = decltype(nc)::value;
        hipLaunchKernelGGL((sample_talker_wave_kernel<T, NC>), dim3(1), dim3(256), 0, s, st, lg, V, seen, G, tf);
    });
    else hipLaunchKernelGGL((sample_talker_kernel<T>), dim3(1), dim3(256), 0, s, st, lg, V, seen, G, tf);
}
template <typename T>
static void launch_sample_api(fq3_ctx* c, const T* lg, int V, const SampleCfg& cfg, const int64_t* history, int n_hist,
                              const T* noise, int64_t* out, hipStream_t s) {
    if (cfg.top_p >= 1.0f) {
        const unsigned char* seen = nullptr;
        if (n_hist > 0) {
            hipLaunchKernelGGL(build_seen_kernel, dim3(1), dim3(256), 0, s, history, n_hist, c->seen_api, V);
            seen = c->seen_api;
        }
        dispatch_nc(V, [&](auto nc) {
            constexpr int NC = decltype(nc)::value;
            hipLaunchKernelGGL((sample_api_wave_kernel<T, NC>), dim3(1), dim3(256), 0, s, lg, V, cfg, seen, noise, out);
        });
    } else {
        hipLaunchKernelGGL((sample_api_kernel<T>), dim3(1), dim3(256), 0, s, lg, V, cfg, history, n_hist, noise, out);
    }
}

static SampleCfg to_cfg(const fq3_sampling& s) {
    SampleCfg c{};
    c.temperature = s.temperature; c.top_k = s.top_k; c.top_p = s.top_p; c.do_sample = s.do_sample;
    c.rep_penalty = s.repetition_penalty; c.sup_lo = 0; c.sup_hi = 0; c.keep_id = -1; c.sup_extra = -1;
    return c;
}

extern "C" int fq3_sample(fq3_ctx* c, const void* logits, int V, const fq3_sampling* sp, const int64_t* history,
                          int n_hist, int sup_lo, int sup_hi, int keep_id, int suppress_eos, const void* noise,
                          int64_t* out_token, void* stream) {
    if (!c || !logits || !sp || !out_token) return fail(FQ3_EINVAL, "null argument");
    if (V <= 0 || V > kMaxVocab || V % 8) return fail(FQ3_EUNSUPPORTED, "vocab must be a multiple of 8 and at most 4096");
    if (sp->do_sample && !noise) return fail(FQ3_EINVAL, "do_sample needs a noise vector");
    if (sp->do_sample && !(sp->temperature > 0.f)) return fail(FQ3_EINVAL, "temperature must be > 0");
    SampleCfg cfg = to_cfg(*sp);
    cfg.sup_lo = sup_lo; cfg.sup_hi = sup_hi; cfg.keep_id = keep_id;
    cfg.sup_extra = suppress_eos ? c->cfg.codec_eos_token_id : -1;
    hipStream_t s = (hipStream_t)stream;
    if (c->cfg.dtype == FQ3_BF16)
        launch_sample_api<bf16_t>(c, (const bf16_t*)logits, V, cfg, history, history ? n_hist : 0, (const bf16_t*)noise, out_token, s);
    else
        launch_sample_api<float>(c, (const float*)logits, V, cfg, history, history ? n_hist : 0, (const float*)noise, out_token, s);
    LAUNCH_CHECK();
    return FQ3_OK;
}

template <typename T>
__global__ __launch_bounds__(256) void rep_penalty_kernel(T* logits, int V, const unsigned char* seen, float penalty) {
    for (int i = threadIdx.x; i < V; i += 256) {
        if (!seen[i]) continue;
        const float v = DT<T>::ld(logits + i);
        DT<T>::st(logits + i, v > 0.f ? v / penalty : v * penalty);
    }
}
extern "C" int fq3_apply_repetition_penalty(fq3_ctx* c, void* logits, int V, const int64_t* history, int n_hist,
                                            float penalty, void* stream) {
    if (!c || !logits) return fail(FQ3_EINVAL, "null argument");
    if (V <= 0 || V > kMaxVocab) return fail(FQ3_EUNSUPPORTED, "vocab must be at most 4096");
    if (penalty == 1.0f || n_hist <= 0 || !history) return FQ3_OK;
    hipStream_t s = (hipStream_t)stream;
    hipLaunchKernelGGL(build_seen_kernel, dim3(1), dim3(256), 0, s, history, n_hist, c->seen_api, V);
    if (c->cfg.dtype == FQ3_BF16) hipLaunchKernelGGL((rep_penalty_kernel<bf16_t>), dim3(1), dim3(256), 0, s, (bf16_t*)logits, V, c->seen_api, penalty);
    else hipLaunchKernelGGL((rep_penalty_kernel<float>), dim3(1), dim3(256), 0, s, (float*)logits, V, c->seen_api, penalty);
    LAUNCH_CHECK();
    return FQ3_OK;
}

extern "C" int fq3_set_predictor_sampling(fq3_ctx* c, const fq3_sampling* s) {
    if (!c || !s) return fail(FQ3_EINVAL, "null argument");
    if (s->do_sample && !(s->temperature > 0.f)) return fail(FQ3_EINVAL, "temperature must be > 0");
    if ((s->top_p >= 1.0f) != (c->pred_sampling.top_p >= 1.0f)) fq3_graph_reset(c);
    c->pred_sampling = *s;
    return FQ3_OK;
}

template <typename T>
static int predictor_passes_t(fq3_ctx* c, const DecodeState* st_dev, const void* pred_input, const void* noise_imm,
                              int64_t* out64, void* out_logits, hipStream_t s) {
    const fq3_stack_dims &p = c->cfg.predictor, &t = c->cfg.talker;
    const int G = c->cfg.num_code_groups, Vp = p.vocab, Ht = t.hidden;
    SampleCfg scfg = to_cfg(c->pred_sampling);
    for (int pass = 0; pass < G; ++pass) {
        const void* hsrc = c->h;
        if (pass == 0 && c->opt_m2) {
            const T* xa = (const T*)pred_input;
            const T* xb = (const T*)pred_input + Ht;
            if (c->cfg.has_projection) {
                GemvArgs g{};
                g.W = c->wt.proj_w; g.bias = c->wt.proj_b; g.N = p.hidden; g.K = Ht; g.x = xa; g.x2 = xb; g.y = c->pred_x; g.y2 = c->pred_x2;
                if (int r = launch_gemv2<PRO_PLAIN, EPI_STORE>(c, g, s)) return r;
                xa = (const T*)c->pred_x; xb = (const T*)c->pred_x2;
            }
            if (int r = run_predictor_pair(c, xa, xb, s)) return r;
            pass = 1;
            hsrc = c->h2;
        } else {
        const T* x_talker = pass < 2 ? (const T*)pred_input + (size_t)pass * Ht : (const T*)c->pred_next;
        const void* x0 = x_talker;
        if (c->cfg.has_projection) {
            GemvArgs g{};
            g.W = c->wt.proj_w; g.bias = c->wt.proj_b; g.N = p.hidden; g.K = Ht; g.x = x_talker; g.y = c->pred_x;
            if (int r = launch_gemv<PRO_PLAIN, EPI_STORE>(c, g, false, s)) return r;
            x0 = c->pred_x;
        }
        StepSrc src{x0, nullptr, pass};
        src.kv_only_tail = pass == 0;
        if (int r = run_stack(c, false, src, s)) return r;
        }
        if (pass == 0) continue;
        const int cb = pass - 1;
        T* lg = out_logits ? (T*)out_logits + (size_t)cb * Vp : (T*)c->plogits + (size_t)cb * Vp;
        GemvArgs hgm{};
        hgm.eps = p.rms_eps; hgm.W = c->lmh[cb]; hgm.N = Vp; hgm.K = p.hidden; hgm.x = hsrc;
        hgm.norm_w = c->wt.predictor_final_norm; hgm.y = lg;
        if (int r = launch_gemv<PRO_NORM, EPI_STORE>(c, hgm, false, s)) return r;
        const T* nz = noise_imm ? (const T*)noise_imm + (size_t)cb * Vp : nullptr;
        const T* next_emb = cb + 1 < G - 1 ? (const T*)c->pemb[cb] : nullptr;
        launch_sample_pred<T>(st_dev, (const T*)lg, Vp, cb, scfg, nz, st_dev ? c->codes : nullptr, G, out64, next_emb,
                              (T*)c->pred_next, Ht, c->pred_sampling.top_p >= 1.0f, st_dev ? c->tf : nullptr, s);
    }
    return 0;
}

extern "C" int fq3_predictor_loop(fq3_ctx* c, const void* pred_input, const void* noise, int64_t* out_ids,
                                  void* out_logits, void* stream) {
    NEED_BOUND(c);
    if (!pred_input || !out_ids) return fail(FQ3_EINVAL, "null argument");
    if (c->pred_sampling.do_sample && !noise) return fail(FQ3_EINVAL, "predictor sampling enabled but no noise given");
    hipStream_t s = (hipStream_t)stream;
    int r = c->cfg.dtype == FQ3_BF16 ? predictor_passes_t<bf16_t>(c, nullptr, pred_input, noise, out_ids, out_logits, s)
                                     : predictor_passes_t<float>(c, nullptr, pred_input, noise, out_ids, out_logits, s);
    if (r) return r;
    LAUNCH_CHECK();
    return FQ3_OK;
}

__global__ __launch_bounds__(256) void decode_arm_kernel(DecodeState* st, DecodeState init, unsigned char* seen, int seen_bytes,
                                                         uint32_t* past_hidden, const uint32_t* ph_src, int ph_words) {
    for (int i = threadIdx.x; i < seen_bytes / 4; i += 256) reinterpret_cast<uint32_t*>(seen)[i] = 0u;
    for (int i = threadIdx.x; i < ph_words; i += 256) past_hidden[i] = ph_src[i];
    if (threadIdx.x == 0) *st = init;
}
__global__ void decode_set_forced_kernel(TeacherForcing* tf, const int* forced, int* decisions) {
    tf->forced = forced; tf->decisions = decisions;
}

extern "C" int fq3_decode_begin(fq3_ctx* c, const fq3_decode_params* p, void* stream) {
    NEED_BOUND(c);
    if (!p || !p->past_hidden || !p->tts_pad_embed) return fail(FQ3_EINVAL, "null argument");
    if (p->trailing_len > 0 && !p->trailing_text) return fail(FQ3_EINVAL, "trailing_text");
    if (p->talker.do_sample && (!p->talker_noise || p->noise_frames <= 0)) return fail(FQ3_EINVAL, "talker sampling needs a noise ring");
    if (c->pred_sampling.do_sample && (!p->pred_noise || p->noise_frames <= 0)) return fail(FQ3_EINVAL, "predictor sampling needs a noise ring");
    if (p->talker.do_sample && !(p->talker.temperature > 0.f)) return fail(FQ3_EINVAL, "temperature must be > 0");
    if (p->max_new_tokens > c->cfg.max_frames) return fail(FQ3_EINVAL, "max_new_tokens exceeds the context's max_frames");
    if (p->prefill_len <= 0 || p->prefill_len > c->cfg.max_seq_len) return fail(FQ3_EINVAL, "prefill_len");
    if (p->first_token < 0 || p->first_token >= c->cfg.talker.vocab) return fail(FQ3_EINVAL, "first_token outside the codec vocabulary");
    if (p->gen_step < 0 || p->min_new_tokens < 0 || p->max_new_tokens < 0) return fail(FQ3_EINVAL, "negative counters");
    const bool wave = p->talker.top_p >= 1.0f;
    if (wave != c->talker_wave) { fq3_graph_reset(c); c->talker_wave = wave; }
    hipStream_t s = (hipStream_t)stream;
    if (int r = fq3_kv_ensure_(c, p->prefill_len + p->max_new_tokens + 1, s)) return r;
    DecodeState h{};
    h.token = p->first_token; h.frame = 0; h.pos = p->prefill_len; h.gen_step = p->gen_step; h.done = 0; h.text_open = 0;
    h.min_new = p->min_new_tokens; h.max_new = p->max_new_tokens; h.trailing_len = p->trailing_len;
    h.noise_frames = p->noise_frames > 0 ? p->noise_frames : 1;
    h.eos_id = c->cfg.codec_eos_token_id; h.max_seq = c->cfg.max_seq_len;
    h.n_pad = c->n_pad; h.rope_delta = c->rope_delta;
    h.sup_lo = c->cfg.talker.vocab - 1024 > 0 ? c->cfg.talker.vocab - 1024 : 0; h.sup_hi = c->cfg.talker.vocab;
    h.t_temperature = p->talker.temperature; h.t_top_k = p->talker.top_k; h.t_top_p = p->talker.top_p;
    h.t_do_sample = p->talker.do_sample; h.t_rep_penalty = p->talker.repetition_penalty;
    h.p_temperature = c->pred_sampling.temperature; h.p_top_k = c->pred_sampling.top_k; h.p_top_p = c->pred_sampling.top_p;
    h.p_do_sample = c->pred_sampling.do_sample;
    h.trailing_text = p->trailing_text; h.tts_pad = p->tts_pad_embed; h.talker_noise = p->talker_noise; h.pred_noise = p->pred_noise;
    hipLaunchKernelGGL(decode_arm_kernel, dim3(1), dim3(256), 0, s, c->st, h, c->seen, (int)kMaxVocab,
                       (uint32_t*)c->past_hidden, (const uint32_t*)p->past_hidden, (int)((size_t)c->cfg.talker.hidden * c->esz / 4));
    LAUNCH_CHECK();
    c->armed = true; c->tt_open = false; c->tt_session = false; c->tt_rows = 0; c->tt_cap = 0;
    c->begin_trailing = p->trailing_text; c->begin_trailing_len = p->trailing_len > 0 ? p->trailing_len : 0;
    return FQ3_OK;
}

__global__ void decode_cancel_kernel(DecodeState* st) { st->done = 1; }
extern "C" int fq3_decode_cancel(fq3_ctx* c, void* stream) {
    if (!c) return fail(FQ3_EINVAL, "null ctx");
    hipLaunchKernelGGL(decode_cancel_kernel, dim3(1), dim3(1), 0, (hipStream_t)stream, c->st);
    LAUNCH_CHECK();
    return FQ3_OK;
}

extern "C" int fq3_decode_set_forced(fq3_ctx* c, const int32_t* forced_codes, int32_t* decisions, void* stream) {
    NEED_BOUND(c);
    if (!c->tf) {
        if (!forced_codes && !decisions) return FQ3_OK;
        if (int r = dmalloc(c, (void**)&c->tf, sizeof(TeacherForcing))) return r;
        fq3_graph_reset(c);
    }
    hipLaunchKernelGGL(decode_set_forced_kernel, dim3(1), dim3(1), 0, (hipStream_t)stream, c->tf, forced_codes, decisions);
    LAUNCH_CHECK();
    return FQ3_OK;
}

template <typename T>
static int enqueue_frame_t(fq3_ctx* c, hipStream_t s) {
    const fq3_stack_dims& t = c->cfg.talker;
    const int G = c->cfg.num_code_groups, H = t.hidden;
    DecodeState* st = c->st;
    hipLaunchKernelGGL((frame_begin_kernel<T>), dim3(1), dim3(256), 0, s, st, (const T*)c->wt.codec_embedding,
                       (const T*)c->past_hidden, (T*)c->ph_hold, (T*)c->pred_in, c->codes, c->seen, H, G);
    if (int r = predictor_passes_t<T>(c, st, c->pred_in, nullptr, nullptr, nullptr, s)) return r;
    EmbTables tabs{};
    tabs.t[0] = c->wt.codec_embedding;
    for (int i = 1; i < G; ++i) tabs.t[i] = c->pemb[i - 1];
    if (G != 16) return fail(FQ3_EUNSUPPORTED, "the fused loop is built for 16 code groups");
    hipLaunchKernelGGL((embed_sum_kernel<T, 16>), dim3(1), dim3(256), 0, s, st, tabs, c->codes, (T*)c->xin, H,
                       c->wt.talker_cos, c->wt.talker_sin, c->wt.talker_rope_len, c->rope_delta, c->rope_now);
    StepSrc src{c->xin, &st->pos, 0};
    if (int r = run_stack(c, true, src, s)) return r;
    GemvArgs g{};
    g.eps = t.rms_eps; g.W = c->wt.codec_head; g.N = t.vocab; g.K = H; g.x = c->h;
    g.norm_w = c->wt.talker_final_norm; g.y = c->logits; g.xn_out = c->past_hidden;
    if (int r = launch_gemv<PRO_NORM, EPI_STORE>(c, g, true, s)) return r;
    launch_sample_talker<T>(st, (const T*)c->logits, t.vocab, c->seen, G, c->talker_wave, c->tf, s);
    return 0;
}
static int enqueue_frame(fq3_ctx* c, hipStream_t s) {
    return c->cfg.dtype == FQ3_BF16 ? enqueue_frame_t<bf16_t>(c, s) : enqueue_frame_t<float>(c, s);
}

extern "C" int fq3_graph_capture(fq3_ctx* c, void* stream) {
    NEED_BOUND(c);
    if (c->exec) return FQ3_OK;
    (void)stream;
    hipStream_t cs = c->cap_stream;
    HIPCHK(hipStreamBeginCapture(cs, hipStreamCaptureModeRelaxed));
    int r = enqueue_frame(c, cs);
    hipGraph_t g = nullptr;
    hipError_t e = hipStreamEndCapture(cs, &g);
    if (r) { if (g) (void)hipGraphDestroy(g); return r; }
    if (e != hipSuccess) return fail(FQ3_EHIP, std::string("hipStreamEndCapture: ") + hipGetErrorString(e));
    c->graph = g;
    HIPCHK(hipGraphInstantiate(&c->exec, c->graph, nullptr, nullptr, 0));
    return FQ3_OK;
}

extern "C" int fq3_decode_frames(fq3_ctx* c, int n_frames, void* stream) {
    NEED_BOUND(c);
    hipStream_t s = (hipStream_t)stream;
    for (int i = 0; i < n_frames; ++i) {
        if (c->exec) { HIPCHK(hipGraphLaunch(c->exec, s)); }
        else if (int r = enqueue_frame(c, s)) return r;
    }
    LAUNCH_CHECK();
    return FQ3_OK;
}

extern "C" int fq3_decode_poll(fq3_ctx* c, int* n_frames_total, int* done, void* stream) {
    if (!c) return fail(FQ3_EINVAL, "null ctx");
    hipStream_t s = (hipStream_t)stream;
    DecodeState h;
    HIPCHK(hipMemcpyAsync(&h, c->st, sizeof h, hipMemcpyDeviceToHost, s));
    HIPCHK(hipStreamSynchronize(s));
    if (n_frames_total) *n_frames_total = h.frame;
    if (done) *done = h.done == 2 ? 2 : (h.done || h.token == h.eos_id);
    return FQ3_OK;
}

__global__ void codes_to_i64_kernel(const int* src, int64_t* dst, int n) {
    const int i = blockIdx.x * blockDim.x + threadIdx.x;
    if (i < n) dst[i] = src[i];
}

extern "C" int fq3_decode_codes(fq3_ctx* c, int from, int count, int64_t* out, void* stream) {
    if (!c || !out) return fail(FQ3_EINVAL, "null argument");
    if (from < 0 || count < 0 || from + count > c->cfg.max_frames) return fail(FQ3_EINVAL, "range");
    const int G = c->cfg.num_code_groups, n = count * G;
    if (n == 0) return FQ3_OK;
    hipLaunchKernelGGL(codes_to_i64_kernel, dim3((n + 255) / 256), dim3(256), 0, (hipStream_t)stream,
                       c->codes + (size_t)from * G, out, n);
    LAUNCH_CHECK();
    return FQ3_OK;
}
```

faster-qwen3-tts_amd/csrc/fq3_ctx.h:

```cpp
#pragma once
#include "../../include/fq3hip.h"
#include "decode_kernels.cuh"
#include <hip/hip_runtime.h>
#include <mutex>
#include <string>
#include <utility>
#include <vector>

struct fq3_kv_pool {
    int dtype = 0, esz = 2, n_layers = 0, n_kv = 0, n_blocks = 0;
    size_t blk_elems = 0;
    std::vector<void*> k, v;
    std::vector<int> free_list;
    std::mutex mu;
    int in_use_high = 0;
    int users = 0;
    bool is_private = false;
};

struct StackBufs {
    std::vector<void*> k, v;
    int max_seq = 0, workers = 1;
    fq3_kv_pool* pool = nullptr;
    int* d_table = nullptr;
    std::vector<int> blocks;
    int max_blocks = 0;
};

struct fq3_ctx {
    fq3_config cfg{};
    int esz = 2;
    std::vector<fq3_layer_weights> tl, pl;
    fq3_weight_table wt{};
    std::vector<const void*> pemb, lmh;
    const void** d_pemb = nullptr;
    bool bound = false;
    StackBufs tk, pk;
    void *h = nullptr, *xin = nullptr, *qkv = nullptr, *act = nullptr, *logits = nullptr, *past_hidden = nullptr;
    void *pred_in = nullptr, *pred_x = nullptr, *pred_next = nullptr, *plogits = nullptr, *tmp_hidden = nullptr;
    void *attn_out = nullptr, *attn_out2 = nullptr;
    void *h2 = nullptr, *qkv2 = nullptr, *act2 = nullptr, *pred_x2 = nullptr;
    size_t part_stride = 0;
    float* part = nullptr;
    float* rope_now = nullptr;
    unsigned char* seen_api = nullptr;
    fq3::DecodeState* st = nullptr;
    fq3::TeacherForcing* tf = nullptr;
    unsigned char* seen = nullptr;
    int* codes = nullptr;
    int64_t* ids64 = nullptr;
    int n_pad = 0, rope_delta = 0;
    int opt_nt = 1;
    int opt_m2 = 1;
    int opt_pred_attn = 1;
    int opt_rmax = 2;
    int opt_flash_prefill = 1;
    int opt_flash_small = 1;
    int opt_swiglu_tile = 1;
    int opt_packed = 1;
    std::vector<std::pair<const void*, int>> packed_refs;
    int opt_no_skinny = 0;
    int prefill_mode = 0;
    bool talker_wave = true;
    fq3_sampling pred_sampling{0.9f, 50, 1.0f, 1, 1.0f};
    hipGraph_t graph = nullptr;
    hipGraphExec_t exec = nullptr;
    hipStream_t cap_stream = nullptr;
    std::vector<void*> allocs;
    fq3_prompt_weights pw{};
    bool pw_bound = false;
    void *pw_x = nullptr, *pw_h = nullptr;
    int pw_cap = 0;
    void* ph_hold = nullptr;
    void *tt_tab = nullptr, *tt_x = nullptr, *tt_h = nullptr;
    int tt_alloc = 0;
    int tt_cap = 0, tt_rows = 0;
    bool tt_open = false, tt_session = false;
    bool armed = false;
    const void* begin_trailing = nullptr; int begin_trailing_len = 0;
    void *pf_x = nullptr, *pf_xn = nullptr, *pf_qkv = nullptr, *pf_att = nullptr, *pf_gu = nullptr, *pf_act = nullptr, *pf_ws = nullptr;
};


const void* fq3_packed_find_(const void* W, int kind);
int fq3_packed_acquire_(const void* W, int N, int K, int kind);
void fq3_packed_release_(const void* W, int kind);

int fq3_fail_(int code, const std::string& m);
int fq3_kv_ensure_(fq3_ctx* c, int n_pos, hipStream_t s);
int fq3_prefill_reserve_(fq3_ctx* c);
int fq3_prefill_mfma_(fq3_ctx* c, const void* embeds, int L, int n_pad, void* out_logits, void* out_hidden, hipStream_t s);
int fq3_prefill_batch_mfma_(fq3_ctx* const* cs, int n, const void* const* embeds, const int* L, const int* n_pad, void* const* out_logits,
                            void* const* out_hidden, hipStream_t s);
int fq3_codec_head_launch_(fq3_ctx* c, const void* hidden, void* out_logits, hipStream_t s);
int fq3_dmalloc_(fq3_ctx* c, void** p, size_t bytes);
void fq3_text_project_launch_(fq3_ctx* c, const int64_t* ids, int n, void* x, void* h, void* out, hipStream_t s);
```

faster-qwen3-tts_amd/csrc/sampler_wave.cuh:

```cuda
#pragma once
#include "sampler.cuh"

namespace fq3 {

__device__ __forceinline__ ArgMax wave_argmax(ArgMax a) {
    ArgMax r;
    r.v = wave_max(a.v);
    r.i = wave_min_i32(a.v == r.v ? a.i : 0x7fffffff);
    return r;
}

struct BlkSmem { int cnt[2][4]; float f[4]; float av[4]; int ai[4]; };

__device__ __forceinline__ float blk_max4(float v, BlkSmem& sm) {
    v = wave_max(v);
    __syncthreads();
    if ((threadIdx.x & 63) == 0) sm.f[threadIdx.x >> 6] = v;
    __syncthreads();
    return fmaxf(fmaxf(sm.f[0], sm.f[1]), fmaxf(sm.f[2], sm.f[3]));
}
__device__ __forceinline__ float blk_sum4(float v, BlkSmem& sm) {
    v = wave_sum(v);
    __syncthreads();
    if ((threadIdx.x & 63) == 0) sm.f[threadIdx.x >> 6] = v;
    __syncthreads();
    return (sm.f[0] + sm.f[1]) + (sm.f[2] + sm.f[3]);
}
__device__ __forceinline__ int blk_argmax4(ArgMax a, BlkSmem& sm) {
    a = wave_argmax(a);
    __syncthreads();
    if ((threadIdx.x & 63) == 0) { sm.av[threadIdx.x >> 6] = a.v; sm.ai[threadIdx.x >> 6] = a.i; }
    __syncthreads();
    ArgMax r; r.v = sm.av[0]; r.i = sm.ai[0];
#pragma unroll
    for (int i = 1; i < 4; ++i) { ArgMax b; b.v = sm.av[i]; b.i = sm.ai[i]; r = amax2(r, b); }
    return r.i;
}

template <typename T, int NC>
__device__ int sample_wave_core(Raw8<T> (&xraw)[NC], int V, const SampleCfg& c, const unsigned char* seen,
                                const T* noise, BlkSmem& sm) {
    const int tid = threadIdx.x;
    float x[NC][8];
    Raw8<T> nz[NC];
    const bool samp = c.do_sample != 0;
#pragma unroll
    for (int j = 0; j < NC; ++j) {
        const int off = j * 2048 + tid * 8;
        if (samp && off < V) ldraw<false>(nz[j], noise + off); else zero(nz[j]);
    }
    const bool pen = seen && c.rep_penalty != 1.0f;
#pragma unroll
    for (int j = 0; j < NC; ++j) {
        const int off = j * 2048 + tid * 8;
        unpack(xraw[j], x[j]);
        unsigned long long sb = 0ull;
        if (pen && off < V) sb = *reinterpret_cast<const unsigned long long*>(seen + off);
#pragma unroll
        for (int i = 0; i < 8; ++i) {
            const int id = off + i;
            float v = x[j][i];
            if (pen && ((sb >> (8 * i)) & 0xffull)) v = v > 0.f ? DT<T>::rnd(v / c.rep_penalty) : DT<T>::rnd(v * c.rep_penalty);
            if (id >= V || (id >= c.sup_lo && id < c.sup_hi && id != c.keep_id) || id == c.sup_extra) v = -INFINITY;
            x[j][i] = v;
        }
    }
    if (!samp) {
        ArgMax a; a.v = -INFINITY; a.i = 0x7fffffff;
#pragma unroll
        for (int j = 0; j < NC; ++j)
#pragma unroll
            for (int i = 0; i < 8; ++i) { ArgMax b; b.v = x[j][i]; b.i = j * 2048 + tid * 8 + i; a = amax2(a, b); }
        return blk_argmax4(a, sm);
    }
#pragma unroll
    for (int j = 0; j < NC; ++j)
#pragma unroll
        for (int i = 0; i < 8; ++i) x[j][i] = DT<T>::rnd(x[j][i] / c.temperature);
    if (c.top_k > 0) {
        const int kk = min(c.top_k, V);
        uint32_t key[NC][8];
#pragma unroll
        for (int j = 0; j < NC; ++j)
#pragma unroll
            for (int i = 0; i < 8; ++i) key[j][i] = (j * 2048 + tid * 8 + i) < V ? okey(x[j][i]) : 0u;
        uint32_t prefix = 0;
        constexpr int kLowBit = sizeof(T) == 2 ? 16 : 0;
        const int wave = tid >> 6;
#pragma unroll 1
        for (int bit = 31; bit >= kLowBit; --bit) {
            const uint32_t cand = prefix | (1u << bit);
            int cnt = 0;
#pragma unroll
            for (int j = 0; j < NC; ++j)
#pragma unroll
                for (int i = 0; i < 8; ++i) cnt += __popcll(__ballot(key[j][i] >= cand));
            int* slot = sm.cnt[bit & 1];
            if ((tid & 63) == 0) slot[wave] = cnt;
            __syncthreads();
            const int tot = (slot[0] + slot[1]) + (slot[2] + slot[3]);
            if (tot >= kk) prefix = cand;
            if (tot == kk) break;
        }
#pragma unroll
        for (int j = 0; j < NC; ++j)
#pragma unroll
            for (int i = 0; i < 8; ++i)
                if (key[j][i] < prefix) x[j][i] = -INFINITY;
    }
    float mx = -INFINITY;
#pragma unroll
    for (int j = 0; j < NC; ++j)
#pragma unroll
        for (int i = 0; i < 8; ++i) mx = fmaxf(mx, x[j][i]);
    mx = blk_max4(mx, sm);
    float se = 0.f;
#pragma unroll
    for (int j = 0; j < NC; ++j)
#pragma unroll
        for (int i = 0; i < 8; ++i) { x[j][i] = expf(x[j][i] - mx); se += x[j][i]; }
    se = blk_sum4(se, sm);
    ArgMax a; a.v = -INFINITY; a.i = 0x7fffffff;
#pragma unroll
    for (int j = 0; j < NC; ++j) {
        float q[8];
        unpack(nz[j], q);
#pragma unroll
        for (int i = 0; i < 8; ++i) {
            const int id = j * 2048 + tid * 8 + i;
            const float p = DT<T>::rnd(x[j][i] / se);
            ArgMax b; b.v = id < V ? DT<T>::rnd(p / q[i]) : -INFINITY; b.i = id;
            a = amax2(a, b);
        }
    }
    return blk_argmax4(a, sm);
}

template <typename T, int NC>
__device__ __forceinline__ void issue_logits(Raw8<T> (&xraw)[NC], const T* logits, int V) {
#pragma unroll
    for (int j = 0; j < NC; ++j) {
        const int off = j * 2048 + threadIdx.x * 8;
        if (off < V) ldraw<false>(xraw[j], logits + off); else zero(xraw[j]);
    }
}

template <typename T, int NC>
__global__ __launch_bounds__(256) void sample_api_wave_kernel(const T* logits, int V, SampleCfg c, const unsigned char* seen,
                                                             const T* noise, int64_t* out) {
    __shared__ BlkSmem sm;
    Raw8<T> xraw[NC];
    issue_logits<T, NC>(xraw, logits, V);
    const int tok = sample_wave_core<T, NC>(xraw, V, c, seen, noise, sm);
    if (threadIdx.x == 0) out[0] = tok;
}

template <typename T, int NC>
__device__ __forceinline__ int sample_nucleus_from_regs(Raw8<T> (&xraw)[NC], int V, const SampleCfg& c, const unsigned char* seen,
                                                        const T* noise, SampleSmem& big) {
#pragma unroll
    for (int j = 0; j < NC; ++j) {
        float f[8];
        unpack(xraw[j], f);
#pragma unroll
        for (int i = 0; i < 8; ++i) {
            const int id = j * 2048 + threadIdx.x * 8 + i;
            if (id < V) big.vals[id] = f[i];
        }
    }
    __syncthreads();
    const int tok = sample_core<T>(big, V, c, seen, noise);
    __syncthreads();
    return tok;
}

template <typename T, int NC, bool NUCLEUS = false>
__device__ __forceinline__ void sample_pred_wave_body(const DecodeState* st, const T* logits, int V, int cb,
                                                      const SampleCfg& c_imm, const T* noise_imm, int* codes, int G,
                                                      int64_t* out64, const T* next_emb, T* next_in, int H, const TeacherForcing* tf = nullptr) {
    __shared__ BlkSmem sm;
    Raw8<T> xraw[NC];
    issue_logits<T, NC>(xraw, logits, V);
    SampleCfg c = c_imm;
    const T* noise = noise_imm;
    int frame = 0;
    if (st) {
        if (st->done) return;
        c.temperature = st->p_temperature; c.top_k = st->p_top_k; c.top_p = st->p_top_p; c.do_sample = st->p_do_sample;
        frame = st->frame;
        if (st->pred_noise)
            noise = gptr(reinterpret_cast<const T*>(st->pred_noise)) + ((size_t)(frame % st->noise_frames) * (G - 1) + cb) * V;
    }
    int tok;
    if constexpr (NUCLEUS) {
        __shared__ SampleSmem big;
        if (c.do_sample && c.top_p < 1.0f) tok = sample_nucleus_from_regs<T, NC>(xraw, V, c, nullptr, noise, big);
        else tok = sample_wave_core<T, NC>(xraw, V, c, nullptr, noise, sm);
    } else {
        tok = sample_wave_core<T, NC>(xraw, V, c, nullptr, noise, sm);
    }
    if (st) tok = forced_or(tf, frame * G + 1 + cb, tok);
    if (threadIdx.x == 0) {
        if (codes) codes[(size_t)frame * G + 1 + cb] = tok;
        if (out64) out64[cb] = tok;
    }
    if (next_emb) {
        const T* src = next_emb + (size_t)tok * H;
        for (int e = threadIdx.x * 8; e < H; e += 256 * 8) {
            Raw8<T> r; ldraw<false>(r, src + e);
            if (sizeof(T) == 2) *reinterpret_cast<u32x4*>(reinterpret_cast<char*>(next_in) + (size_t)e * 2) = *reinterpret_cast<u32x4*>(&r);
            else { float f[8]; unpack(r, f);
#pragma unroll
                   for (int i = 0; i < 8; ++i) DT<T>::st(next_in + e + i, f[i]); }
        }
    }
}

template <typename T, int NC>
__global__ __launch_bounds__(256) void sample_pred_wave_kernel(const DecodeState* st, const T* logits, int V, int cb,
                                                              SampleCfg c_imm, const T* noise_imm, int* codes, int G,
                                                              int64_t* out64, const T* next_emb, T* next_in, int H, const TeacherForcing* tf) {
    sample_pred_wave_body<T, NC>(st, logits, V, cb, c_imm, noise_imm, codes, G, out64, next_emb, next_in, H, tf);
}

template <typename T, int NC, bool NUCLEUS = false>
__device__ __forceinline__ void sample_talker_wave_body(DecodeState* st, const T* logits, int V, const unsigned char* seen, int G,
                                                        const TeacherForcing* tf = nullptr) {
    __shared__ BlkSmem sm;
    Raw8<T> xraw[NC];
    issue_logits<T, NC>(xraw, logits, V);
    if (st->done) return;
    SampleCfg c;
    c.temperature = st->t_temperature; c.top_k = st->t_top_k; c.top_p = st->t_top_p; c.do_sample = st->t_do_sample;
    c.rep_penalty = st->t_rep_penalty;
    c.sup_lo = st->sup_lo; c.sup_hi = st->sup_hi; c.keep_id = st->eos_id;
    const int frame = st->frame;
    c.sup_extra = (frame + 1 < st->min_new) ? st->eos_id : -1;
    const T* noise = st->talker_noise
        ? gptr(reinterpret_cast<const T*>(st->talker_noise)) + (size_t)(frame % st->noise_frames) * V : nullptr;
    int tok;
    if constexpr (NUCLEUS) {
        __shared__ SampleSmem big;
        if (c.do_sample && c.top_p < 1.0f) tok = sample_nucleus_from_regs<T, NC>(xraw, V, c, seen, noise, big);
        else tok = sample_wave_core<T, NC>(xraw, V, c, seen, noise, sm);
    } else {
        tok = sample_wave_core<T, NC>(xraw, V, c, seen, noise, sm);
    }
    tok = forced_or(tf, (frame + 1) * G, tok);
    if (threadIdx.x == 0) { st->token = tok; st->frame = frame + 1; st->pos += 1; st->gen_step += 1; }
}
template <typename T, int NC>
__global__ __launch_bounds__(256) void sample_talker_wave_kernel(DecodeState* st, const T* logits, int V,
                                                                const unsigned char* seen, int G, const TeacherForcing* tf) {
    sample_talker_wave_body<T, NC>(st, logits, V, seen, G, tf);
}

}
```

Before: 36.88.

## Precompute predictor layer-0 QKV per codebook token and fuse sampling with attention

Adds a per-codebook table holding the code predictor's layer-0 normed QKV projection for every vocabulary token, built once at bind time and shared across contexts. A sampled token then selects its QKV row directly, so the layer-0 QKV GEMV is skipped for later passes. For small positions the sampler kernel also runs the next pass's layer-0 attention itself, and the first two predictor positions are merged into one pair attention launch. This trades extra device memory and a one-time table build for fewer launches and less GEMV work per codebook step; sampling blocks redundantly recompute the token in every block.

```diff
diff --git a/faster-qwen3-tts_amd/csrc/decode_kernels.cuh b/faster-qwen3-tts_amd/csrc/decode_kernels.cuh
--- a/faster-qwen3-tts_amd/csrc/decode_kernels.cuh
+++ b/faster-qwen3-tts_amd/csrc/decode_kernels.cuh
@@ -415,8 +415,14 @@
 template <typename T, int REP, bool PAGED>
 __global__ __launch_bounds__(256) void attn_decode_kernel(AttnArgs a) { attn_decode_body<T, REP, PAGED>(a); }
 
-template <typename T>
-__device__ __forceinline__ void attn_pred_body(const AttnArgs& a, int head) {
+struct AttnPairSrc {
+    const void* qkv_a;
+    const float* cos_a; const float* sin_a;
+    void* out_a;
+};
+
+template <typename T, bool PAIR = false>
+__device__ __forceinline__ void attn_pred_body(const AttnArgs& a, int head, const AttnPairSrc* pa = nullptr) {
     constexpr int HD = kHeadDim;
     const int g = head / a.rep, hh = head - g * a.rep;
     const int lane = threadIdx.x & 63, sub = lane >> 4, c = lane & 15;
@@ -433,8 +439,18 @@
     ldraw<false>(kwraw, reinterpret_cast<const T*>(a.k_norm_w) + c * 8);
     const f32x4 cs0 = *reinterpret_cast<const f32x4*>(a.cos_row + ((c * 8) & 63)), cs1 = *reinterpret_cast<const f32x4*>(a.cos_row + ((c * 8 + 4) & 63));
     const f32x4 sn0 = *reinterpret_cast<const f32x4*>(a.sin_row + ((c * 8) & 63)), sn1 = *reinterpret_cast<const f32x4*>(a.sin_row + ((c * 8 + 4) & 63));
+    Raw8<T> karaw, varaw;
+    f32x4 ca0, ca1, sa0, sa1;
+    if constexpr (PAIR) {
+        const T* qa = reinterpret_cast<const T*>(pa->qkv_a);
+        ldraw<false>(karaw, qa + q_dim + (size_t)g * HD + c * 8);
+        ldraw<false>(varaw, qa + q_dim + kv_dim + (size_t)g * HD + c * 8);
+        ca0 = *reinterpret_cast<const f32x4*>(pa->cos_a + ((c * 8) & 63)); ca1 = *reinterpret_cast<const f32x4*>(pa->cos_a + ((c * 8 + 4) & 63));
+        sa0 = *reinterpret_cast<const f32x4*>(pa->sin_a + ((c * 8) & 63)); sa1 = *reinterpret_cast<const f32x4*>(pa->sin_a + ((c * 8 + 4) & 63));
+    }
 #pragma unroll
     for (int i = 0; i < 4; ++i) {
+        if constexpr (PAIR) { zero(kr[i]); zero(vr[i]); continue; }
         int key = i * 4 + sub;
         key = key < a.max_seq ? key : a.max_seq - 1;
         ldraw<false>(kr[i], kc + (size_t)key * HD + c * 8);
@@ -444,7 +460,7 @@
     const float sgn = c < 8 ? -1.f : 1.f;
     const float cs[8] = {cs0.x, cs0.y, cs0.z, cs0.w, cs1.x, cs1.y, cs1.z, cs1.w};
     const float sn[8] = {sgn * sn0.x, sgn * sn0.y, sgn * sn0.z, sgn * sn0.w, sgn * sn1.x, sgn * sn1.y, sgn * sn1.z, sgn * sn1.w};
-    auto norm_rope = [&](const Raw8<T>& raw, const Raw8<T>& wraw, float (&out)[8]) {
+    auto norm_rope = [&](const Raw8<T>& raw, const Raw8<T>& wraw, const float (&cs)[8], const float (&sn)[8], float (&out)[8]) {
         float x[8], w[8];
         unpack(raw, x); unpack(wraw, w);
         float ss = 0.f;
@@ -471,18 +487,39 @@
         }
     };
     float qr[8], knew[8], vnew[8];
-    norm_rope(qraw, qwraw, qr);
-    norm_rope(knraw, kwraw, knew);
+    norm_rope(qraw, qwraw, cs, sn, qr);
+    norm_rope(knraw, kwraw, cs, sn, knew);
     unpack(vnraw, vnew);
     if (hh == 0 && sub == 0) {
         DT<T>::st8(kc + (size_t)pos * HD + c * 8, knew);
         DT<T>::st8(vc + (size_t)pos * HD + c * 8, vnew);
     }
+    float ka[8], va[8];
+    if constexpr (PAIR) {
+        const float csa[8] = {ca0.x, ca0.y, ca0.z, ca0.w, ca1.x, ca1.y, ca1.z, ca1.w};
+        const float sna[8] = {sgn * sa0.x, sgn * sa0.y, sgn * sa0.z, sgn * sa0.w, sgn * sa1.x, sgn * sa1.y, sgn * sa1.z, sgn * sa1.w};
+        norm_rope(karaw, kwraw, csa, sna, ka);
+        unpack(varaw, va);
+        if (sub == 0) {
+            if (hh == 0) {
+                DT<T>::st8(kc + c * 8, ka);
+                DT<T>::st8(vc + c * 8, va);
+            }
+            float oa[8];
+#pragma unroll
+            for (int d = 0; d < 8; ++d) oa[d] = va[d] + 0.f;
+            DT<T>::st8(reinterpret_cast<T*>(pa->out_a) + (size_t)head * HD + c * 8, oa);
+        }
+    }
     float sc[5];
 #pragma unroll
     for (int i = 0; i < 4; ++i) {
         float kf[8], s = 0.f;
         unpack(kr[i], kf);
+        if constexpr (PAIR) if (i == 0 && sub == 0) {
+#pragma unroll
+            for (int d = 0; d < 8; ++d) kf[d] = ka[d];
+        }
 #pragma unroll
         for (int d = 0; d < 8; ++d) s = fmaf(qr[d], kf[d], s);
         s = row16_sum(s);
@@ -507,6 +544,10 @@
         float vf[8];
         if (!(i * 4 + sub < pos)) zero(vr[i]);
         unpack(vr[i], vf);
+        if constexpr (PAIR) if (i == 0 && sub == 0) {
+#pragma unroll
+            for (int d = 0; d < 8; ++d) vf[d] = va[d];
+        }
 #pragma unroll
         for (int d = 0; d < 8; ++d) o[d] = fmaf(p[i], vf[d], o[d]);
     }
@@ -628,6 +669,8 @@
 
 template <typename T>
 __global__ __launch_bounds__(64) void attn_pred_kernel(AttnArgs a) { attn_pred_body<T>(a); }
+template <typename T>
+__global__ __launch_bounds__(64) void attn_pred_pair_kernel(AttnArgs a, AttnPairSrc pa) { attn_pred_body<T, true>(a, (int)blockIdx.x, &pa); }
 
 template <typename T>
 __global__ __launch_bounds__(256) void rmsnorm_kernel(const T* x, const T* w, T* y, int K, float eps) {
@@ -659,10 +702,10 @@
 
 struct TeacherForcing { const int* forced; int* decisions; };
 
-__device__ __forceinline__ int forced_or(const TeacherForcing* tf, int slot, int tok) {
+__device__ __forceinline__ int forced_or(const TeacherForcing* tf, int slot, int tok, bool record = true) {
     if (!tf) return tok;
     const int* forced = gptr(tf->forced); int* dec = gptr(tf->decisions);
-    if (dec && threadIdx.x == 0) dec[slot] = tok;
+    if (dec && record && threadIdx.x == 0) dec[slot] = tok;
     return forced ? forced[slot] : tok;
 }
 
diff --git a/faster-qwen3-tts_amd/csrc/fq3_api.hip b/faster-qwen3-tts_amd/csrc/fq3_api.hip
--- a/faster-qwen3-tts_amd/csrc/fq3_api.hip
+++ b/faster-qwen3-tts_amd/csrc/fq3_api.hip
@@ -9,6 +9,7 @@
 #include <cstring>
 #include <map>
 #include <string>
+#include <tuple>
 #include <type_traits>
 #include <vector>
 
@@ -243,9 +244,26 @@
     return FQ3_OK;
 }
 
+static int pred_lean_effective(const fq3_ctx* c) {
+    const bool tab = (c->opt_pred_lean & 1) && c->opt_pred_attn && c->qkv_tab && c->pred_sampling.top_p >= 1.0f;
+    int m = tab ? 1 : 0;
+    if ((c->opt_pred_lean & 2) && c->opt_pred_attn && c->opt_m2) m |= 2;
+    if (tab && (c->opt_pred_lean & 4) && c->cfg.predictor.n_heads % 4 == 0) m |= 4;
+    return m;
+}
+static int qkv_table_count();
+
 extern "C" int fq3_set_option(fq3_ctx* c, const char* key, int value) {
     if (!c || !key) return fail(FQ3_EINVAL, "null argument");
     const std::string k(key);
+    if (k == "pred_lean_active") {
+        const int m = pred_lean_effective(c);
+        return m == value ? FQ3_OK : fail(FQ3_ESTATE, "pred_lean: the launches left out are those of mask " + std::to_string(m) + (c->qkv_tab ? "" : " (no layer-0 qkv table)"));
+    }
+    if (k == "pred_lean_tables") {
+        const int n = qkv_table_count();
+        return n == value ? FQ3_OK : fail(FQ3_ESTATE, "pred_lean: " + std::to_string(n) + " layer-0 qkv table(s) in the registry");
+    }
     if (k == "weight_nt") c->opt_nt = value;
     else if (k == "pred_m2") c->opt_m2 = value;
     else if (k == "pred_attn") c->opt_pred_attn = value;
@@ -256,6 +274,7 @@
     else if (k == "swiglu_tile") c->opt_swiglu_tile = value;
     else if (k == "packed_weights") c->opt_packed = value;
     else if (k == "skinny_gemm") c->opt_no_skinny = !value;
+    else if (k == "pred_lean") c->opt_pred_lean = value;
     else return fail(FQ3_EINVAL, "unknown option: " + k);
     fq3_graph_reset(c);
     return FQ3_OK;
@@ -330,11 +349,96 @@
     return FQ3_OK;
 }
 
+template <typename T, int NCH, int PRO>
+__global__ __launch_bounds__(256) void gemv_rows_kernel(GemvArgs a, size_t x_stride, size_t y_stride) {
+    a.x = reinterpret_cast<const T*>(a.x) + blockIdx.y * x_stride;
+    a.y = reinterpret_cast<T*>(a.y) + blockIdx.y * y_stride;
+    gemv_body<T, NCH, PRO, EPI_STORE, false, 1, 1>(a);
+}
+template <typename T, int PRO>
+static bool launch_gemv_rows(const GemvArgs& a, int rows, size_t x_stride, size_t y_stride) {
+    const int n = gemv_chunks(a.K, 4);
+    if (!n) return false;
+    with_value<1, 2, 4>(n, [&](auto nch) {
+        hipLaunchKernelGGL((gemv_rows_kernel<T, decltype(nch)::value, PRO>), dim3((a.N + 3) / 4, rows), dim3(256), 0, nullptr, a, x_stride, y_stride);
+    });
+    return true;
+}
+namespace {
+typedef std::vector<const void*> QkvTabKey;
+struct QkvTabEntry { void* p; int refs; };
+std::mutex g_qkvtab_mu;
+std::map<QkvTabKey, QkvTabEntry> g_qkvtab;
+}
+template <typename T>
+static int qkv_table_build(const fq3_ctx* c, T* tab) {
+    const fq3_stack_dims &p = c->cfg.predictor, &t = c->cfg.talker;
+    const int Vp = p.vocab, N = (p.n_heads + 2 * p.n_kv_heads) * kHeadDim, n_tab = c->cfg.num_code_groups - 2;
+    T* px = nullptr;
+    if (c->cfg.has_projection && hipMalloc((void**)&px, (size_t)Vp * p.hidden * sizeof(T)) != hipSuccess) { (void)hipGetLastError(); return 1; }
+    bool ok = true;
+    for (int cb = 0; cb < n_tab && ok; ++cb) {
+        const T* x = reinterpret_cast<const T*>(c->pemb[cb]);
+        size_t xs = t.hidden;
+        if (c->cfg.has_projection) {
+            GemvArgs g{};
+            g.W = c->wt.proj_w; g.bias = c->wt.proj_b; g.N = p.hidden; g.K = t.hidden; g.x = x; g.y = px;
+            ok = launch_gemv_rows<T, PRO_PLAIN>(g, Vp, xs, p.hidden);
+            x = px; xs = p.hidden;
+        }
+        GemvArgs g{};
+        g.eps = p.rms_eps; g.W = c->pl[0].qkv; g.N = N; g.K = p.hidden; g.x = x; g.norm_w = c->pl[0].input_norm;
+        g.y = tab + (size_t)cb * Vp * N;
+        ok = ok && launch_gemv_rows<T, PRO_NORM>(g, Vp, xs, N);
+    }
+    ok = hipStreamSynchronize(nullptr) == hipSuccess && hipGetLastError() == hipSuccess && ok;
+    if (px) (void)hipFree(px);
+    return ok ? 0 : 2;
+}
+static int qkv_table_count() { std::lock_guard<std::mutex> lk(g_qkvtab_mu); return (int)g_qkvtab.size(); }
+static void qkv_table_release(fq3_ctx* c) {
+    if (!c->qkv_tab) return;
+    std::lock_guard<std::mutex> lk(g_qkvtab_mu);
+    auto it = g_qkvtab.find(c->qkv_tab_key);
+    if (it != g_qkvtab.end() && --it->second.refs <= 0) { (void)hipFree(it->second.p); g_qkvtab.erase(it); }
+    c->qkv_tab = nullptr;
+}
+static int qkv_table_acquire(fq3_ctx* c) {
+    const fq3_stack_dims& p = c->cfg.predictor;
+    const int n_tab = c->cfg.num_code_groups - 2;
+    if (n_tab < 1) return FQ3_OK;
+    QkvTabKey key(c->pemb.begin(), c->pemb.begin() + n_tab);
+    uint32_t eps_bits;
+    memcpy(&eps_bits, &p.rms_eps, sizeof eps_bits);
+    for (const void* q : {c->pl[0].qkv, c->pl[0].input_norm, c->cfg.has_projection ? c->wt.proj_w : nullptr, c->cfg.has_projection ? c->wt.proj_b : nullptr})
+        key.push_back(q);
+    for (uintptr_t v : {(uintptr_t)c->cfg.dtype, (uintptr_t)p.vocab, (uintptr_t)p.hidden, (uintptr_t)p.n_heads, (uintptr_t)p.n_kv_heads,
+                        (uintptr_t)c->cfg.talker.hidden, (uintptr_t)eps_bits})
+        key.push_back(reinterpret_cast<const void*>(v));
+    std::lock_guard<std::mutex> lk(g_qkvtab_mu);
+    auto it = g_qkvtab.find(key);
+    if (it == g_qkvtab.end()) {
+        void* tab = nullptr;
+        const size_t bytes = (size_t)n_tab * p.vocab * (p.n_heads + 2 * p.n_kv_heads) * kHeadDim * c->esz;
+        if (hipMalloc(&tab, bytes) != hipSuccess) { (void)hipGetLastError(); return FQ3_OK; }
+        const int st = c->cfg.dtype == FQ3_BF16 ? qkv_table_build<bf16_t>(c, (bf16_t*)tab) : qkv_table_build<float>(c, (float*)tab);
+        if (st) (void)hipFree(tab);
+        if (st == 1) return FQ3_OK;
+        if (st) return fail(FQ3_EHIP, "building the code predictor's layer-0 qkv table failed");
+        it = g_qkvtab.emplace(key, QkvTabEntry{tab, 0}).first;
+    }
+    ++it->second.refs;
+    c->qkv_tab = it->second.p;
+    c->qkv_tab_key = key;
+    return FQ3_OK;
+}
+
 extern "C" int fq3_ctx_destroy(fq3_ctx* c) {
     if (!c) return FQ3_OK;
     (void)hipDeviceSynchronize();
     fq3_graph_reset(c);
     packed_release_all(c);
+    qkv_table_release(c);
     if (c->cap_stream) (void)hipStreamDestroy(c->cap_stream);
     if (fq3_kv_pool* p = c->tk.pool) {
         (void)fq3_kv_release(c, 0);
@@ -369,7 +473,9 @@
     HIPCHK(hipMemcpy(c->d_pemb, c->pemb.data(), (G - 1) * sizeof(void*), hipMemcpyHostToDevice));
     (void)hipDeviceSynchronize();
     packed_release_all(c);
+    qkv_table_release(c);
     if (int r = packed_acquire_all(c)) { packed_release_all(c); return r; }
+    if (int r = qkv_table_acquire(c)) { packed_release_all(c); return r; }
     c->bound = true;
     fq3_graph_reset(c);
     return FQ3_OK;
@@ -431,7 +537,8 @@
     if (a.table) launch_attn_p<T, true>(a, rep, workers, s); else launch_attn_p<T, false>(a, rep, workers, s);
 }
 
-struct StepSrc { const void* x0; const int* pos_ptr; int pos_imm; bool kv_only_tail = false; };
+static bool pred_one_wave_pos(int pos) { return pos <= 16; }
+struct StepSrc { const void* x0; const int* pos_ptr; int pos_imm; bool kv_only_tail = false; bool qkv_ready = false; bool attn_ready = false; };
 
 static int run_stack(fq3_ctx* c, bool talker, const StepSrc& src, hipStream_t s) {
     const fq3_stack_dims& d = talker ? c->cfg.talker : c->cfg.predictor;
@@ -456,7 +563,8 @@
         g.eps = d.rms_eps;
         g.W = w.qkv; g.N = q_dim + 2 * kv_dim; g.K = d.hidden; g.x = xin;
         g.norm_w = w.input_norm; g.y = c->qkv;
-        if (int r = launch_gemv<PRO_NORM, EPI_STORE>(c, g, nt, s)) return r;
+        if (!(i == 0 && src.qkv_ready))
+            if (int r = launch_gemv<PRO_NORM, EPI_STORE>(c, g, nt, s)) return r;
         const bool tail_skip = src.kv_only_tail && i == d.n_layers - 1;
         GemvArgs o{};
         o.W = w.o; o.N = d.hidden; o.K = q_dim; o.y = c->h; o.res = xin; o.rep = rep;
@@ -471,9 +579,10 @@
         a.n_kv = d.n_kv_heads; a.part = c->part;
         a.scale = 1.0f / sqrtf((float)kHeadDim);
         a.rep = rep; a.out = c->attn_out;
-        const bool pred_attn = c->opt_pred_attn && !talker && !src.pos_ptr && src.pos_imm <= 16;
+        const bool pred_attn = c->opt_pred_attn && !talker && !src.pos_ptr && pred_one_wave_pos(src.pos_imm);
         if (pred_attn) {
-            if (c->cfg.dtype == FQ3_BF16) hipLaunchKernelGGL((attn_pred_kernel<bf16_t>), dim3(d.n_heads), dim3(64), 0, s, a);
+            if (i == 0 && src.attn_ready) {}
+            else if (c->cfg.dtype == FQ3_BF16) hipLaunchKernelGGL((attn_pred_kernel<bf16_t>), dim3(d.n_heads), dim3(64), 0, s, a);
             else hipLaunchKernelGGL((attn_pred_kernel<float>), dim3(d.n_heads), dim3(64), 0, s, a);
             if (tail_skip) break;
             o.x = c->attn_out;
@@ -509,7 +618,8 @@
         g.eps = d.rms_eps; g.W = w.qkv; g.N = q_dim + 2 * kv_dim; g.K = d.hidden; g.x = xa; g.x2 = xb;
         g.norm_w = w.input_norm; g.y = c->qkv; g.y2 = c->qkv2;
         if (int r = launch_gemv2<PRO_NORM, EPI_STORE>(c, g, s)) return r;
-        for (int m = 0; m < 2; ++m) {
+        const bool one_launch = (pred_lean_effective(c) & 2) != 0;
+        for (int m = one_launch ? 1 : 0; m < 2; ++m) {
             AttnArgs a{};
             a.qkv = m == 0 ? c->qkv : c->qkv2; a.q_norm_w = w.q_norm; a.k_norm_w = w.k_norm; a.eps = d.rms_eps;
             a.cos_row = c->wt.pred_cos + (size_t)m * 64; a.sin_row = c->wt.pred_sin + (size_t)m * 64;
@@ -517,7 +627,11 @@
             a.pos_ptr = nullptr; a.pos_imm = m; a.n_pad = 0; a.n_kv = d.n_kv_heads;
             a.part = c->part + (size_t)m * c->part_stride; a.scale = 1.0f / sqrtf((float)kHeadDim);
             a.rep = rep; a.out = m == 0 ? c->attn_out : c->attn_out2;
-            if (c->opt_pred_attn) {
+            if (one_launch) {
+                const AttnPairSrc pa{c->qkv, c->wt.pred_cos, c->wt.pred_sin, c->attn_out};
+                if (c->cfg.dtype == FQ3_BF16) hipLaunchKernelGGL((attn_pred_pair_kernel<bf16_t>), dim3(d.n_heads), dim3(64), 0, s, a, pa);
+                else hipLaunchKernelGGL((attn_pred_pair_kernel<float>), dim3(d.n_heads), dim3(64), 0, s, a, pa);
+            } else if (c->opt_pred_attn) {
                 if (c->cfg.dtype == FQ3_BF16) hipLaunchKernelGGL((attn_pred_kernel<bf16_t>), dim3(d.n_heads), dim3(64), 0, s, a);
                 else hipLaunchKernelGGL((attn_pred_kernel<float>), dim3(d.n_heads), dim3(64), 0, s, a);
             } else if (c->cfg.dtype == FQ3_BF16) launch_attn_t<bf16_t>(a, rep, kv.workers, s);
@@ -795,11 +909,13 @@
 template <typename T>
 static void launch_sample_pred(const DecodeState* st, const T* lg, int V, int cb, const SampleCfg& cfg, const T* nz,
                                int* codes, int G, int64_t* out64, const T* next_emb, T* next_in, int H, bool wave,
-                               const TeacherForcing* tf, hipStream_t s) {
+                               const TeacherForcing* tf, const T* qkv_tab, T* qkv_out, int n_qkv, const AttnArgs* next_attn, hipStream_t s) {
     if (wave) dispatch_nc(V, [&](auto nc) {
         constexpr int NC = decltype(nc)::value;
-        hipLaunchKernelGGL((sample_pred_wave_kernel<T, NC>), dim3(1), dim3(256), 0, s, st, lg, V, cb, cfg, nz, codes, G,
-                           out64, next_emb, next_in, H, tf);
+        if (next_attn) hipLaunchKernelGGL((sample_pred_attn_kernel<T, NC>), dim3(next_attn->n_kv * next_attn->rep / 4), dim3(256), 0, s, st, lg, V, cb, cfg,
+                                          nz, codes, G, out64, next_emb, next_in, H, tf, qkv_tab, n_qkv, *next_attn);
+        else hipLaunchKernelGGL((sample_pred_wave_kernel<T, NC>), dim3(1), dim3(256), 0, s, st, lg, V, cb, cfg, nz, codes, G,
+                           out64, next_emb, next_in, H, tf, qkv_tab, qkv_out, n_qkv);
     });
     else hipLaunchKernelGGL((sample_pred_kernel<T>), dim3(1), dim3(256), 0, s, st, lg, V, cb, cfg, nz, codes, G, out64,
                             next_emb, next_in, H, tf);
@@ -892,6 +1008,11 @@
     const fq3_stack_dims &p = c->cfg.predictor, &t = c->cfg.talker;
     const int G = c->cfg.num_code_groups, Vp = p.vocab, Ht = t.hidden;
     SampleCfg scfg = to_cfg(c->pred_sampling);
+    const bool wave = c->pred_sampling.top_p >= 1.0f;
+    const int lean = pred_lean_effective(c);
+    const bool use_tab = (lean & 1) != 0;
+    const int n_qkv = (p.n_heads + 2 * p.n_kv_heads) * kHeadDim;
+    const bool merge_attn = (lean & 4) != 0;
     for (int pass = 0; pass < G; ++pass) {
         const void* hsrc = c->h;
         if (pass == 0 && c->opt_m2) {
@@ -917,6 +1038,8 @@
         }
         StepSrc src{x0, nullptr, pass};
         src.kv_only_tail = pass == 0;
+        src.qkv_ready = use_tab && pass >= 2;
+        src.attn_ready = merge_attn && pass >= 2 && pred_one_wave_pos(pass);
         if (int r = run_stack(c, false, src, s)) return r;
         }
         if (pass == 0) continue;
@@ -928,8 +1051,19 @@
         if (int r = launch_gemv<PRO_NORM, EPI_STORE>(c, hgm, false, s)) return r;
         const T* nz = noise_imm ? (const T*)noise_imm + (size_t)cb * Vp : nullptr;
         const T* next_emb = cb + 1 < G - 1 ? (const T*)c->pemb[cb] : nullptr;
+        const T* tab = use_tab && next_emb ? (const T*)c->qkv_tab + (size_t)cb * Vp * n_qkv : nullptr;
+        AttnArgs na{};
+        const bool merge_here = tab && merge_attn && pred_one_wave_pos(pass + 1);
+        if (merge_here) {
+            const int pos = pass + 1, rp = pos < c->wt.pred_rope_len ? pos : c->wt.pred_rope_len - 1;
+            na.q_norm_w = c->pl[0].q_norm; na.k_norm_w = c->pl[0].k_norm; na.eps = p.rms_eps;
+            na.cos_row = c->wt.pred_cos + (size_t)rp * 64; na.sin_row = c->wt.pred_sin + (size_t)rp * 64;
+            na.kcache = c->pk.k[0]; na.vcache = c->pk.v[0]; na.max_seq = c->pk.max_seq;
+            na.pos_imm = pos; na.n_kv = p.n_kv_heads; na.part = c->part; na.scale = 1.0f / sqrtf((float)kHeadDim);
+            na.rep = p.n_heads / p.n_kv_heads; na.out = c->attn_out;
+        }
         launch_sample_pred<T>(st_dev, (const T*)lg, Vp, cb, scfg, nz, st_dev ? c->codes : nullptr, G, out64, next_emb,
-                              (T*)c->pred_next, Ht, c->pred_sampling.top_p >= 1.0f, st_dev ? c->tf : nullptr, s);
+                              (T*)c->pred_next, Ht, wave, st_dev ? c->tf : nullptr, tab, (T*)c->qkv, n_qkv, merge_here ? &na : nullptr, s);
     }
     return 0;
 }
diff --git a/faster-qwen3-tts_amd/csrc/fq3_ctx.h b/faster-qwen3-tts_amd/csrc/fq3_ctx.h
--- a/faster-qwen3-tts_amd/csrc/fq3_ctx.h
+++ b/faster-qwen3-tts_amd/csrc/fq3_ctx.h
@@ -59,6 +59,9 @@
     int opt_swiglu_tile = 1;
     int opt_packed = 1;
     std::vector<std::pair<const void*, int>> packed_refs;
+    int opt_pred_lean = 7;
+    const void* qkv_tab = nullptr;
+    std::vector<const void*> qkv_tab_key;
     int opt_no_skinny = 0;
     int prefill_mode = 0;
     bool talker_wave = true;
@@ -86,6 +89,7 @@
 int fq3_packed_acquire_(const void* W, int N, int K, int kind);
 void fq3_packed_release_(const void* W, int kind);
 
+
 int fq3_fail_(int code, const std::string& m);
 int fq3_kv_ensure_(fq3_ctx* c, int n_pos, hipStream_t s);
 int fq3_prefill_reserve_(fq3_ctx* c);
diff --git a/faster-qwen3-tts_amd/csrc/sampler_wave.cuh b/faster-qwen3-tts_amd/csrc/sampler_wave.cuh
--- a/faster-qwen3-tts_amd/csrc/sampler_wave.cuh
+++ b/faster-qwen3-tts_amd/csrc/sampler_wave.cuh
@@ -174,10 +174,27 @@
     return tok;
 }
 
+__device__ __forceinline__ void st_raw(bf16_t* p, const Raw8<bf16_t>& r) { *reinterpret_cast<u32x4*>(p) = r.v; }
+__device__ __forceinline__ void st_raw(float* p, const Raw8<float>& r) { reinterpret_cast<f32x4*>(p)[0] = r.a; reinterpret_cast<f32x4*>(p)[1] = r.b; }
+template <typename T>
+__device__ __forceinline__ void stage_next_pass(const T* emb_row, T* next_in, int H, const T* qkv_row, T* qkv_out, int n_qkv) {
+    const int e0 = threadIdx.x * 8;
+    Raw8<T> re, rq[2];
+    if (e0 < H) ldraw<false>(re, emb_row + e0);
+#pragma unroll
+    for (int k = 0; k < 2; ++k) if (e0 + k * 2048 < n_qkv) ldraw<false>(rq[k], qkv_row + e0 + k * 2048);
+    if (e0 < H) st_raw(next_in + e0, re);
+#pragma unroll
+    for (int k = 0; k < 2; ++k) if (e0 + k * 2048 < n_qkv) st_raw(qkv_out + e0 + k * 2048, rq[k]);
+    for (int e = e0 + 2048; e < H; e += 2048) { ldraw<false>(re, emb_row + e); st_raw(next_in + e, re); }
+    for (int e = e0 + 4096; e < n_qkv; e += 2048) { ldraw<false>(re, qkv_row + e); st_raw(qkv_out + e, re); }
+}
+
 template <typename T, int NC, bool NUCLEUS = false>
-__device__ __forceinline__ void sample_pred_wave_body(const DecodeState* st, const T* logits, int V, int cb,
+__device__ __forceinline__ int sample_pred_wave_body(const DecodeState* st, const T* logits, int V, int cb,
                                                       const SampleCfg& c_imm, const T* noise_imm, int* codes, int G,
-                                                      int64_t* out64, const T* next_emb, T* next_in, int H, const TeacherForcing* tf = nullptr) {
+                                                      int64_t* out64, const T* next_emb, T* next_in, int H, const TeacherForcing* tf = nullptr,
+                                                      const T* qkv_tab = nullptr, T* qkv_out = nullptr, int n_qkv = 0, bool lead = true) {
     __shared__ BlkSmem sm;
     Raw8<T> xraw[NC];
     issue_logits<T, NC>(xraw, logits, V);
@@ -185,7 +202,7 @@
     const T* noise = noise_imm;
     int frame = 0;
     if (st) {
-        if (st->done) return;
+        if (st->done) return -1;
         c.temperature = st->p_temperature; c.top_k = st->p_top_k; c.top_p = st->p_top_p; c.do_sample = st->p_do_sample;
         frame = st->frame;
         if (st->pred_noise)
@@ -199,12 +216,13 @@
     } else {
         tok = sample_wave_core<T, NC>(xraw, V, c, nullptr, noise, sm);
     }
-    if (st) tok = forced_or(tf, frame * G + 1 + cb, tok);
-    if (threadIdx.x == 0) {
+    if (st) tok = forced_or(tf, frame * G + 1 + cb, tok, lead);
+    if (lead && threadIdx.x == 0) {
         if (codes) codes[(size_t)frame * G + 1 + cb] = tok;
         if (out64) out64[cb] = tok;
     }
-    if (next_emb) {
+    if (lead && next_emb && qkv_tab) stage_next_pass<T>(next_emb + (size_t)tok * H, next_in, H, qkv_tab + (size_t)tok * n_qkv, qkv_out, n_qkv);
+    else if (lead && next_emb) {
         const T* src = next_emb + (size_t)tok * H;
         for (int e = threadIdx.x * 8; e < H; e += 256 * 8) {
             Raw8<T> r; ldraw<false>(r, src + e);
@@ -214,13 +232,27 @@
                    for (int i = 0; i < 8; ++i) DT<T>::st(next_in + e + i, f[i]); }
         }
     }
+    return tok;
 }
 
 template <typename T, int NC>
 __global__ __launch_bounds__(256) void sample_pred_wave_kernel(const DecodeState* st, const T* logits, int V, int cb,
                                                               SampleCfg c_imm, const T* noise_imm, int* codes, int G,
-                                                              int64_t* out64, const T* next_emb, T* next_in, int H, const TeacherForcing* tf) {
-    sample_pred_wave_body<T, NC>(st, logits, V, cb, c_imm, noise_imm, codes, G, out64, next_emb, next_in, H, tf);
+                                                              int64_t* out64, const T* next_emb, T* next_in, int H, const TeacherForcing* tf,
+                                                              const T* qkv_tab, T* qkv_out, int n_qkv) {
+    sample_pred_wave_body<T, NC>(st, logits, V, cb, c_imm, noise_imm, codes, G, out64, next_emb, next_in, H, tf, qkv_tab, qkv_out, n_qkv);
+}
+
+template <typename T, int NC>
+__global__ __launch_bounds__(256) void sample_pred_attn_kernel(const DecodeState* st, const T* logits, int V, int cb,
+                                                              SampleCfg c_imm, const T* noise_imm, int* codes, int G,
+                                                              int64_t* out64, const T* next_emb, T* next_in, int H, const TeacherForcing* tf,
+                                                              const T* qkv_tab, int n_qkv, AttnArgs at) {
+    const int tok = sample_pred_wave_body<T, NC>(st, logits, V, cb, c_imm, noise_imm, codes, G, out64, next_emb, next_in, H, tf,
+                                                 (const T*)nullptr, (T*)nullptr, 0, blockIdx.x == 0);
+    if (tok < 0) return;
+    at.qkv = qkv_tab + (size_t)__builtin_amdgcn_readfirstlane(tok) * n_qkv;
+    attn_pred_body<T>(at, (int)blockIdx.x * 4 + (int)(threadIdx.x >> 6));
 }
 
 template <typename T, int NC, bool NUCLEUS = false>
```

New measurement: 38.31 (median of 6 runs). 3.9% higher.
